# isi-vista/VistaOCR

Hardware: AMD Instinct MI355X
Metric: line-images/sec (train, batch 32, 30x600 grey) (higher is better)
Workload: dtype f32 (the LSTM's large GEMMs as bf16x6 products: fp32 operands split exactly into three bf16 planes, six bf16 MFMAs per fp32 product, fp32 accumulate; VOCR_LSTM_GEMM=f32 restores the f32-MFMA kernels); 1 GPU; configs[1]: 32 synthetic 1x30x600 grey lines per GPU, 20 labels/line, V=96, 3xBiLSTM-512, train() = H2D of the batch + fwd+CTC+bwd+allreduce+clamp+Adam, loss returned as a float; widths=600 .. 600 px, mean 600, conv_dtype=fp32, global_batch=32, parallelism=dp1, ranks_seen=1, backend=none, per_rank_rng=seed 1234 + 1000*rank after an identical init

## Files before the change

include/vocr.h:

```cpp
#ifndef VOCR_H
#define VOCR_H
#include <stddef.h>
#include <stdint.h>

#ifdef __cplusplus
extern "C" {
#endif

#define VOCR_OK          0
#define VOCR_EINVAL     -1
#define VOCR_ELAUNCH    -2
#define VOCR_ENODEVICE  -3
#define VOCR_ECOMM      -4


const char* vocr_last_error(void);
#define VOCR_ABI_VERSION 5
int  vocr_abi_version(void);
int  vocr_profile_range_push(const char* name);
int  vocr_profile_range_pop(void);
int  vocr_device_count(void);

int vocr_conv3x3_pack_weights(const float* w, float* wpack_fwd, float* wpack_dgrad, int cout, int cin, void* stream);
int vocr_conv3x3_fwd(const float* x, const float* wpack, const float* bias, float* y,
                     int n, int cin, int h, int w, int cout, void* stream);
size_t vocr_conv3x3_wgrad_workspace_bytes(int n, int cin, int h, int w, int cout);
int vocr_conv3x3_wgrad(const float* x, const float* dy, float* dw, void* workspace,
                       int n, int cin, int h, int w, int cout, void* stream);
int vocr_conv3x3_wino_supported(int cin, int cout);
size_t vocr_conv3x3_wino_pack_floats(int cout, int cin);
int vocr_conv3x3_wino_pack_weights(const float* w, float* wpack_fwd, float* wpack_dgrad, int cout, int cin, void* stream);
int vocr_conv3x3_wino_plan(int n, int cin, int h, int w, int cout);
int vocr_conv3x3_wino_fwd(const float* x, const float* wpack, const float* bias, float* y,
                          int n, int cin, int h, int w, int cout, void* stream);
size_t vocr_conv3x3_wgrad_wino_workspace_bytes(int n, int cin, int h, int w, int cout);
int vocr_conv3x3_wgrad_wino(const float* x, const float* dy, float* dw, void* workspace,
                            int n, int cin, int h, int w, int cout, void* stream);
int vocr_conv3x3_c1_fwd(const float* x, const float* w, const float* bias, float* y, int n, int h, int wd, int cout, int round_f16,
                        void* stream);
size_t vocr_conv3x3_c1_wgrad_workspace_bytes(int n, int h, int cout);
int vocr_conv3x3_c1_wgrad(const float* x, const float* dy, float* dw, float* dbias, void* workspace, int n, int h, int wd, int cout,
                          void* stream);
size_t vocr_conv3x3_f16_pack_bytes(int cout, int cin, int dgrad);
int vocr_conv3x3_f16_pack_weights(const float* w, void* wpack_fwd, void* wpack_dgrad, int cout, int cin, void* stream);
int vocr_conv3x3_f16_fwd(const float* x, const void* wpack, const float* bias, float* y,
                         int n, int cin, int h, int w, int cout, void* stream);
int vocr_conv3x3_wgrad_f16(const float* x, const float* dy, float* dw, void* workspace,
                           int n, int cin, int h, int w, int cout, void* stream);
int vocr_conv3x3_h16_supported(int cin, int cout);
int vocr_conv3x3_h16_plan(int n, int cin, int h, int w, int cout);
int vocr_conv3x3_h16_fwd(const void* x16, const void* wpack, const float* bias, float* y,
                         int n, int cin, int h, int w, int cout, void* stream);
int vocr_f16_padded_row(int w);
int vocr_f32_to_f16_layouts(const float* x, void* nhwc, void* nchwp, int n, int c, int h, int w, void* stream);
int vocr_conv3x3_wgrad_h16_supported(int cin, int cout);
size_t vocr_conv3x3_wgrad_h16_workspace_bytes(int n, int cin, int h, int w, int cout);
int vocr_conv3x3_wgrad_h16(const void* x16p, const void* dy16p, float* dw, void* workspace,
                           int n, int cin, int h, int w, int cout, void* stream);
size_t vocr_channel_sum_workspace_bytes(int n, int c, int hw);
int vocr_channel_sum(const float* x, float* out, int n, int c, int hw, void* workspace, void* stream);

size_t vocr_bn_workspace_bytes(int n, int c, int hw);
int vocr_bn_train_stats(const float* y, int n, int c, int hw, float eps, float momentum,
                        float* mean, float* invstd, float* running_mean, float* running_var,
                        int64_t* num_batches_tracked, float* xhat_sum, void* workspace, void* stream);
int vocr_bn_eval_stats(const float* running_mean, const float* running_var, int c, float eps,
                       float* mean, float* invstd, void* stream);
int vocr_bn_relu_apply(const float* y, const float* mean, const float* invstd, const float* gamma,
                       const float* beta, float* out, int n, int c, int hw, void* stream);
int vocr_bn_train_relu_apply(const float* y, const float* gamma, const float* beta, float* out, int n, int c, int hw, float eps,
                             float momentum, float* mean, float* invstd, float* running_mean, float* running_var,
                             int64_t* num_batches_tracked, float* xhat_sum, void* workspace, void* stream);
int vocr_bn_train_relu_fracpool2x2_fwd(const float* y, const float* gamma, const float* beta, const float* samples, float* out,
                                       int32_t* idx, int n, int c, int h, int w, int oh, int ow, float eps, float momentum,
                                       float* mean, float* invstd, float* running_mean, float* running_var,
                                       int64_t* num_batches_tracked, float* xhat_sum, void* workspace, void* stream);
int vocr_bn_relu_bwd(const float* da, const float* y, const float* mean, const float* invstd,
                     const float* gamma, const float* beta, const float* xhat_sum, float* dy, float* dgamma, float* dbeta,
                     float* dconv_bias, int n, int c, int hw, void* workspace, void* stream);

int vocr_fracpool2x2_fwd(const float* x, const float* samples, float* out, int32_t* idx,
                         int n, int c, int h, int w, int oh, int ow, void* stream);
int vocr_bn_relu_fracpool2x2_fwd(const float* y, const float* mean, const float* invstd, const float* gamma,
                                 const float* beta, const float* samples, float* out, int32_t* idx,
                                 int n, int c, int h, int w, int oh, int ow, void* stream);
int vocr_bn_relu_fracpool2x2_bwd_supported(int h, int w, int oh, int ow);
int vocr_bn_relu_fracpool2x2_bwd(const float* dout, const int32_t* idx, const float* samples, const float* y,
                                 const float* mean, const float* invstd, const float* gamma, const float* beta,
                                 const float* xhat_sum, float* dy, float* dgamma, float* dbeta, float* dconv_bias,
                                 int n, int c, int h, int w, int oh, int ow, void* workspace, void* stream);
int vocr_fracpool2x2_bwd(const float* dout, const int32_t* idx, float* dx,
                         int n, int c, int h, int w, int oh, int ow, void* stream);

int vocr_relu_maxpool2_fwd(const float* x, float* out, int32_t* idx, int n, int c, int h, int w, void* stream);
int vocr_relu_maxpool2_bwd(const float* dout, const float* out, const int32_t* idx, float* dx,
                           int n, int c, int h, int w, void* stream);

size_t vocr_gemm_workspace_bytes(int m, int n, int k, int has_bias_or_relu);
int vocr_gemm(int transa, int transb, int m, int n, int k,
              const float* a, int lda, const float* b, int ldb, float* c, int ldc,
              const float* bias, int relu, int accumulate, void* workspace, size_t workspace_bytes, void* stream);
#define VOCR_GEMM_PLAN_INTS 12
int vocr_gemm_plan(int transa, int transb, int m, int n, int k, int lda, int ldb, int ldc, int aligned, int has_bias_or_relu,
                   int accumulate, size_t workspace_bytes, int nprob, int nseg, int tiles_only, int* plan);
size_t vocr_gemm_pair_workspace_bytes(int m, int n, int k, int mode);
int vocr_gemm_pair(int mode, int transa, int transb, int m, int n, int k, const float* a0, const float* a1, int lda,
                   const float* b0, const float* b1, int ldb, float* c0, float* c1, int ldc, const float* bias0, const float* bias1,
                   int relu, void* workspace, size_t workspace_bytes, void* stream);
size_t vocr_colsum_workspace_bytes(int m, int n);
int vocr_colsum(const float* x, float* out, int m, int n, void* workspace, void* stream);
int vocr_relu_bwd(const float* dy, const float* out, float* dz, size_t count, void* stream);
int vocr_bchw_to_wbch(const float* x, float* out, int b, int c, int h, int w, void* stream);
int vocr_wbch_to_bchw(const float* x, float* out, int b, int c, int h, int w, void* stream);
int vocr_mul(const float* x, const float* mask, float* out, size_t count, void* stream);
int vocr_add(const float* x, const float* y, float* out, size_t count, void* stream);
int vocr_scale_dev(const float* x, const float* scalar, float* out, size_t count, void* stream);
int vocr_dropout_fwd(const float* x, float* out, float* mask, size_t count, float p, uint64_t seed, void* stream);
int vocr_dropout_mask(float* mask, size_t count, float p, uint64_t seed, void* stream);

size_t vocr_lstm_workspace_bytes(int t, int b, int h);
int vocr_lstm_fwd(const float* xproj, const float* whh_fwd, const float* whh_rev, const int32_t* lens, float* y,
                  float* gates, float* cell, void* workspace, int t, int b, int h, int32_t* health, void* stream);
int vocr_lstm_fwd_range(const float* xproj, const float* whh_fwd, const float* whh_rev, const int32_t* lens, float* y,
                        float* gates, float* cell, void* workspace, int t, int b, int h, int step_begin, int step_end,
                        int32_t* health, void* stream);
int vocr_lstm_bwd(const float* dy, const float* whht_fwd, const float* whht_rev, const int32_t* lens, const float* gates,
                  const float* cell, float* dgates, void* workspace, int t, int b, int h, int32_t* health, void* stream);
int vocr_lstm_bwd_bias(const float* dy, const float* whht_fwd, const float* whht_rev, const int32_t* lens, const float* gates,
                       const float* cell, float* dgates, float* dbias, void* workspace, int t, int b, int h, int32_t* health,
                       void* stream);
int vocr_lstm_bwd_parts_supported(int t, int b, int h);
int vocr_lstm_bwd_parts(const float* dy, const float* dy_mask, const float* whht_fwd, const float* whht_rev, const int32_t* lens,
                        const float* gates, const float* cell, float* dgates, void* workspace, int t, int b, int h,
                        int32_t* health, void* stream);
int vocr_lstm_bias_from_parts(float* dbias, const void* workspace, int t, int b, int h, void* stream);

size_t vocr_gemm_x6_planes_bytes(int rows, int k);
int vocr_gemm_x6_split(const float* x, const float* x2, int seg, int seg_axis, const float* mask, long ld, int rows, int k, int k_contiguous,
                       void* planes, void* stream);
size_t vocr_gemm_x6_workspace_bytes(int m, int n, int k);
#define VOCR_GEMM_X6_PLAN_INTS 9
int vocr_gemm_x6_plan(int m, int n, int k, int b_rows, int b_row0, int b_row0_2, int has_workspace, int* plan);
int vocr_gemm_x6(const void* a_planes, int a_rows, int a_k, int a_row0, int a_kk0, const void* b_planes, int b_rows, int b_k, int b_row0, int b_kk0,
                 int m, int n, int k, float* c0, float* c1, int csplit, int rsplit, int ldc, const float* bias0, const float* bias1, int relu,
                 void* workspace, void* stream);

int vocr_gemm_x6_two_views(const void* a_planes, int a_rows, int a_k, int a_row0, const void* b_planes, int b_rows, int b_k, int m, int n, int k,
                           int rsplit, int a_kk0, int b_row0, int b_kk0, int a_kk0_2, int b_row0_2, int b_kk0_2, float* c0, float* c1, int ldc,
                           void* workspace, void* stream);

size_t vocr_gemm_h3_planes_bytes(int rows, int k);
int vocr_gemm_h3_split(const float* x, const float* x2, int seg, int seg_axis, const float* mask, long ld, int rows, int k, int k_contiguous,
                       float bound, void* planes, void* stream);
int vocr_gemm_h3(const void* a_planes, int a_rows, int a_k, int a_row0, int a_kk0, const void* b_planes, int b_rows, int b_k, int b_row0, int b_kk0,
                 int m, int n, int k, float* c0, float* c1, int csplit, int rsplit, int ldc, const float* bias0, const float* bias1, int relu,
                 void* workspace, void* stream);
int vocr_gemm_h3_two_views(const void* a_planes, int a_rows, int a_k, int a_row0, const void* b_planes, int b_rows, int b_k, int m, int n, int k,
                           int rsplit, int a_kk0, int b_row0, int b_kk0, int a_kk0_2, int b_row0_2, int b_kk0_2, float* c0, float* c1, int ldc,
                           void* workspace, void* stream);

int vocr_lstm_packed_supported(int b, int h);
int vocr_seq_rowmap(const int32_t* lens, int t, int b, int rows, int32_t* to_packed, int32_t* to_dense, void* stream);
int vocr_gather_rows(const float* src, float* dst, const int32_t* map, long nrows, int n, const float* fill, void* stream);
size_t vocr_gather_rows_fill_grad_workspace_bytes(int n);
int vocr_gather_rows_fill_grad(const float* dout, const int32_t* map, long nrows, int n, float* dfill, void* workspace, void* stream);
int vocr_lstm_fwd_packed(const float* xproj, const float* whh_fwd, const float* whh_rev, const int32_t* lens, float* y,
                         float* gates, float* cell, void* workspace, int t, int b, int h, int rows, int32_t* health, void* stream);
int vocr_lstm_bwd_packed(const float* dy, const float* dy_mask, const float* whht_fwd, const float* whht_rev, const int32_t* lens,
                         const float* gates, const float* cell, float* dgates, float* dbias, void* workspace, int t, int b, int h,
                         int rows, int32_t* health, void* stream);

int vocr_lstm_follow_supported(int b, int h);
size_t vocr_lstm_xproj_pack_bytes(int h);
int vocr_lstm_xproj_pack(const float* w_ih_fwd, const float* w_ih_rev, float* wpack, int h, void* stream);
int vocr_lstm_fwd_lead(const float* xproj, const float* xproj2, const float* whh_fwd, const float* whh_rev, const int32_t* lens,
                       float* y, float* gates, float* cell, void* workspace, int t, int b, int h, int rows,
                       const float* next_wpack, const float* next_bias, const float* y_mask, float* next_planes,
                       int32_t* health, void* stream);

size_t vocr_ctc_workspace_bytes(int t, int b, int v, int max_label_len);
int vocr_ctc_loss_grad(const float* logits, const int32_t* labels, const int32_t* label_offsets,
                       const int32_t* label_lens, const int32_t* act_lens, float* nll, float* dlogits,
                       void* workspace, int t, int b, int v, int max_label_len, void* stream);

int vocr_argmax_rows(const float* x, int32_t* idx, float* maxv, int rows, int v, void* stream);
int vocr_greedy_collapse(const int32_t* idx, const float* maxv, const int32_t* lens, const int32_t* canon,
                         int32_t* out_labels, int32_t* out_counts, int t, int b, float thresh, void* stream);

size_t vocr_ctc_beam_workspace_bytes(int t, int b, int v, int beam, int nbest);
int vocr_ctc_beam_search(const float* logits, const int32_t* lens, int t, int b, int v, const int32_t* canon, int beam, int nbest,
                         const float* lm_logp, const int32_t* lm_next, const float* lm_eos, int lm_states, int lm_start,
                         float lm_weight, float insertion_bonus, float prune_logp, int32_t* out_labels, int32_t* out_lens,
                         float* out_scores, void* workspace, size_t workspace_bytes, void* stream);

size_t vocr_ctc_word_beam_workspace_bytes(int t, int b, int v, int beam, int nbest);
int vocr_ctc_word_beam_search(const float* logits, const int32_t* lens, int t, int b, int v, const int32_t* canon, int beam, int nbest,
                              const int32_t* cls_kind, const int32_t* cls_tok, const int32_t* trie_next, const int32_t* trie_tok,
                              const float* trie_la, int trie_nodes, const int32_t* lm_off, const int32_t* lm_succ_tok,
                              const float* lm_succ_logp, const int32_t* lm_succ_next, const float* lm_bow, const int32_t* lm_back,
                              int lm_states, int lm_succ, int lm_tokens, int lm_start, int tok_unk, int tok_eos, float lm_weight,
                              float word_bonus, float oov_penalty, int32_t* out_labels, int32_t* out_lens, float* out_scores,
                              void* workspace, size_t workspace_bytes, void* stream);

size_t vocr_ctc_align_workspace_bytes(int t, int b, int v, int n, int max_label_len);
int vocr_ctc_align(const float* logits, const int32_t* lens, int t, int b, int v, const int32_t* canon,
                   const int32_t* labels, const int32_t* label_lens, int n, int label_stride, int max_label_len,
                   float* out_scores, int32_t* out_spans, float* out_label_scores,
                   void* workspace, size_t workspace_bytes, void* stream);

size_t vocr_ctc_edit_workspace_bytes(int t, int b, int v, int n, int max_label_len);
int vocr_ctc_edit_scores(const float* logits, const int32_t* lens, int t, int b, int v, const int32_t* canon,
                         const int32_t* labels, const int32_t* label_lens, int n, int label_stride, int max_label_len,
                         float* out_ctc, float* out_sub, float* out_del, float* out_ins,
                         void* workspace, size_t workspace_bytes, void* stream);

size_t vocr_ctc_nbest_workspace_bytes(int t, int b, int v, int n, int max_label_len);
int vocr_ctc_nbest_grad(const float* logits, const int32_t* lens, int t, int b, int v, const int32_t* canon,
                        const int32_t* labels, const int32_t* label_lens, int n, int label_stride, int max_label_len,
                        const float* weights, float* out_ctc, float* dlogits,
                        void* workspace, size_t workspace_bytes, void* stream);

size_t vocr_ctc_keyword_workspace_bytes(int t, int b, int v, int nq, int max_query_len);
int vocr_ctc_keyword_scores(const float* logits, const int32_t* lens, int t, int b, int v, const int32_t* canon,
                            const int32_t* queries, const int32_t* query_lens, const int32_t* query_flags, int nq, int query_stride,
                            int max_query_len, float* out_log_count, float* out_best, int32_t* out_span,
                            void* workspace, size_t workspace_bytes, void* stream);

size_t vocr_ctc_grammar_workspace_bytes(int t, int b, int v, int g, int max_states, int max_arcs, int want_best);
int vocr_ctc_grammar_scores(const float* logits, const int32_t* lens, int t, int b, int v, const int32_t* canon,
// ... 47 lines not shown
```

vistaocr_amd/_lib.py:

```python
import ctypes
import os
from ctypes import c_char_p, c_float, c_int, c_size_t, c_uint32, c_uint64, c_void_p

_HERE = os.path.dirname(os.path.abspath(__file__))
LIB_PATH = os.path.join(_HERE, "csrc", "libvocr.so")

P, I, F, Z, U64, U32 = c_void_p, c_int, c_float, c_size_t, c_uint64, c_uint32

SIGNATURES = {
    "vocr_last_error": (c_char_p, []),
    "vocr_abi_version": (I, []),
    "vocr_device_count": (I, []),
    "vocr_profile_range_push": (I, [c_char_p]),
    "vocr_profile_range_pop": (I, []),
    "vocr_conv3x3_pack_weights": (I, [P, P, P, I, I, P]),
    "vocr_conv3x3_fwd": (I, [P, P, P, P, I, I, I, I, I, P]),
    "vocr_conv3x3_wgrad_workspace_bytes": (Z, [I, I, I, I, I]),
    "vocr_conv3x3_wgrad": (I, [P, P, P, P, I, I, I, I, I, P]),
    "vocr_conv3x3_wino_supported": (I, [I, I]),
    "vocr_conv3x3_wino_pack_floats": (Z, [I, I]),
    "vocr_conv3x3_wino_pack_weights": (I, [P, P, P, I, I, P]),
    "vocr_conv3x3_wino_fwd": (I, [P, P, P, P, I, I, I, I, I, P]),
    "vocr_conv3x3_wino_plan": (I, [I, I, I, I, I]),
    "vocr_conv3x3_wgrad_wino_workspace_bytes": (Z, [I, I, I, I, I]),
    "vocr_conv3x3_wgrad_wino": (I, [P, P, P, P, I, I, I, I, I, P]),
    "vocr_conv3x3_f16_pack_bytes": (Z, [I, I, I]),
    "vocr_conv3x3_f16_pack_weights": (I, [P, P, P, I, I, P]),
    "vocr_conv3x3_f16_fwd": (I, [P, P, P, P, I, I, I, I, I, P]),
    "vocr_conv3x3_wgrad_f16": (I, [P, P, P, P, I, I, I, I, I, P]),
    "vocr_conv3x3_c1_fwd": (I, [P, P, P, P, I, I, I, I, I, P]),
    "vocr_conv3x3_c1_wgrad_workspace_bytes": (Z, [I, I, I]),
    "vocr_conv3x3_c1_wgrad": (I, [P, P, P, P, P, I, I, I, I, P]),
    "vocr_conv3x3_h16_supported": (I, [I, I]),
    "vocr_conv3x3_h16_plan": (I, [I, I, I, I, I]),
    "vocr_conv3x3_h16_fwd": (I, [P, P, P, P, I, I, I, I, I, P]),
    "vocr_f16_padded_row": (I, [I]),
    "vocr_f32_to_f16_layouts": (I, [P, P, P, I, I, I, I, P]),
    "vocr_conv3x3_wgrad_h16_supported": (I, [I, I]),
    "vocr_conv3x3_wgrad_h16_workspace_bytes": (Z, [I, I, I, I, I]),
    "vocr_conv3x3_wgrad_h16": (I, [P, P, P, P, I, I, I, I, I, P]),
    "vocr_channel_sum_workspace_bytes": (Z, [I, I, I]),
    "vocr_channel_sum": (I, [P, P, I, I, I, P, P]),
    "vocr_bn_workspace_bytes": (Z, [I, I, I]),
    "vocr_bn_train_stats": (I, [P, I, I, I, F, F, P, P, P, P, P, P, P, P]),
    "vocr_bn_eval_stats": (I, [P, P, I, F, P, P, P]),
    "vocr_bn_relu_apply": (I, [P, P, P, P, P, P, I, I, I, P]),
    "vocr_bn_train_relu_apply": (I, [P, P, P, P, I, I, I, F, F, P, P, P, P, P, P, P, P]),
    "vocr_bn_train_relu_fracpool2x2_fwd": (I, [P, P, P, P, P, P, I, I, I, I, I, I, F, F, P, P, P, P, P, P, P, P]),
    "vocr_bn_relu_bwd": (I, [P, P, P, P, P, P, P, P, P, P, P, I, I, I, P, P]),
    "vocr_bn_relu_fracpool2x2_bwd_supported": (I, [I, I, I, I]),
    "vocr_bn_relu_fracpool2x2_bwd": (I, [P] * 13 + [I] * 6 + [P, P]),
    "vocr_fracpool2x2_fwd": (I, [P, P, P, P, I, I, I, I, I, I, P]),
    "vocr_bn_relu_fracpool2x2_fwd": (I, [P, P, P, P, P, P, P, P, I, I, I, I, I, I, P]),
    "vocr_fracpool2x2_bwd": (I, [P, P, P, I, I, I, I, I, I, P]),
    "vocr_relu_maxpool2_fwd": (I, [P, P, P, I, I, I, I, P]),
    "vocr_relu_maxpool2_bwd": (I, [P, P, P, P, I, I, I, I, P]),
    "vocr_gemm_workspace_bytes": (Z, [I, I, I, I]),
    "vocr_gemm": (I, [I, I, I, I, I, P, I, P, I, P, I, P, I, I, P, Z, P]),
    "vocr_gemm_plan": (I, [I, I, I, I, I, I, I, I, I, I, I, Z, I, I, I, P]),
    "vocr_gemm_pair_workspace_bytes": (Z, [I, I, I, I]),
    "vocr_gemm_pair": (I, [I, I, I, I, I, I, P, P, I, P, P, I, P, P, I, P, P, I, P, Z, P]),
    "vocr_gemm_x6_planes_bytes": (Z, [I, I]),
    "vocr_gemm_x6_split": (I, [P, P, I, I, P, ctypes.c_long, I, I, I, P, P]),
    "vocr_gemm_x6_workspace_bytes": (Z, [I, I, I]),
    "vocr_gemm_x6_plan": (I, [I, I, I, I, I, I, I, P]),
    "vocr_gemm_x6": (I, [P, I, I, I, I, P, I, I, I, I, I, I, I, P, P, I, I, I, P, P, I, P, P]),
    "vocr_gemm_x6_two_views": (I, [P, I, I, I, P, I, I, I, I, I, I, I, I, I, I, I, I, P, P, I, P, P]),
    "vocr_gemm_h3_two_views": (I, [P, I, I, I, P, I, I, I, I, I, I, I, I, I, I, I, I, P, P, I, P, P]),
    "vocr_gemm_h3_planes_bytes": (Z, [I, I]),
    "vocr_gemm_h3_split": (I, [P, P, I, I, P, ctypes.c_long, I, I, I, ctypes.c_float, P, P]),
    "vocr_gemm_h3": (I, [P, I, I, I, I, P, I, I, I, I, I, I, I, P, P, I, I, I, P, P, I, P, P]),
    "vocr_colsum_workspace_bytes": (Z, [I, I]),
    "vocr_colsum": (I, [P, P, I, I, P, P]),
    "vocr_relu_bwd": (I, [P, P, P, Z, P]),
    "vocr_bchw_to_wbch": (I, [P, P, I, I, I, I, P]),
    "vocr_wbch_to_bchw": (I, [P, P, I, I, I, I, P]),
    "vocr_mul": (I, [P, P, P, Z, P]),
    "vocr_add": (I, [P, P, P, Z, P]),
    "vocr_scale_dev": (I, [P, P, P, Z, P]),
    "vocr_dropout_fwd": (I, [P, P, P, Z, F, U64, P]),
    "vocr_dropout_mask": (I, [P, Z, F, U64, P]),
    "vocr_lstm_workspace_bytes": (Z, [I, I, I]),
    "vocr_lstm_fwd": (I, [P, P, P, P, P, P, P, P, I, I, I, P, P]),
    "vocr_lstm_fwd_range": (I, [P, P, P, P, P, P, P, P, I, I, I, I, I, P, P]),
    "vocr_lstm_bwd": (I, [P, P, P, P, P, P, P, P, I, I, I, P, P]),
    "vocr_lstm_bwd_bias": (I, [P, P, P, P, P, P, P, P, P, I, I, I, P, P]),
    "vocr_lstm_bwd_parts_supported": (I, [I, I, I]),
    "vocr_lstm_bwd_parts": (I, [P, P, P, P, P, P, P, P, P, I, I, I, P, P]),
    "vocr_lstm_bias_from_parts": (I, [P, P, I, I, I, P]),
    "vocr_lstm_packed_supported": (I, [I, I]),
    "vocr_seq_rowmap": (I, [P, I, I, I, P, P, P]),
    "vocr_gather_rows": (I, [P, P, P, ctypes.c_long, I, P, P]),
    "vocr_gather_rows_fill_grad_workspace_bytes": (Z, [I]),
    "vocr_gather_rows_fill_grad": (I, [P, P, ctypes.c_long, I, P, P, P]),
    "vocr_lstm_fwd_packed": (I, [P, P, P, P, P, P, P, P, I, I, I, I, P, P]),
    "vocr_lstm_follow_supported": (I, [I, I]),
    "vocr_lstm_xproj_pack_bytes": (Z, [I]),
    "vocr_lstm_xproj_pack": (I, [P, P, P, I, P]),
    "vocr_lstm_fwd_lead": (I, [P, P, P, P, P, P, P, P, P, I, I, I, I, P, P, P, P, P, P]),
    "vocr_lstm_bwd_packed": (I, [P, P, P, P, P, P, P, P, P, P, I, I, I, I, P, P]),
    "vocr_ctc_workspace_bytes": (Z, [I, I, I, I]),
    "vocr_ctc_loss_grad": (I, [P, P, P, P, P, P, P, P, I, I, I, I, P]),
    "vocr_argmax_rows": (I, [P, P, P, I, I, P]),
    "vocr_greedy_collapse": (I, [P, P, P, P, P, P, I, I, F, P]),
    "vocr_ctc_beam_workspace_bytes": (Z, [I, I, I, I, I]),
    "vocr_ctc_beam_search": (I, [P, P, I, I, I, P, I, I, P, P, P, I, I, F, F, F, P, P, P, P, Z, P]),
    "vocr_ctc_word_beam_workspace_bytes": (Z, [I, I, I, I, I]),
    "vocr_ctc_word_beam_search": (I, [P, P, I, I, I, P, I, I, P, P, P, P, P, I, P, P, P, P, P, P, I, I, I, I, I, I, F, F, F, P, P, P, P,
                                      Z, P]),
    "vocr_ctc_align_workspace_bytes": (Z, [I, I, I, I, I]),
    "vocr_ctc_align": (I, [P, P, I, I, I, P, P, P, I, I, I, P, P, P, P, Z, P]),
    "vocr_ctc_edit_workspace_bytes": (Z, [I, I, I, I, I]),
    "vocr_ctc_edit_scores": (I, [P, P, I, I, I, P, P, P, I, I, I, P, P, P, P, P, Z, P]),
    "vocr_ctc_nbest_workspace_bytes": (Z, [I, I, I, I, I]),
    "vocr_ctc_nbest_grad": (I, [P, P, I, I, I, P, P, P, I, I, I, P, P, P, P, Z, P]),
    "vocr_ctc_keyword_workspace_bytes": (Z, [I, I, I, I, I]),
    "vocr_ctc_keyword_scores": (I, [P, P, I, I, I, P, P, P, P, I, I, I, P, P, P, P, Z, P]),
    "vocr_ctc_grammar_workspace_bytes": (Z, [I, I, I, I, I, I, I]),
    "vocr_ctc_grammar_scores": (I, [P, P, I, I, I, P, P, P, I, P, P, P, P, I, I, P, P, P, P, I, P, Z, P]),
    "vocr_ctc_grammar_grad_workspace_bytes": (Z, [I, I, I, I, I, I, I]),
    "vocr_ctc_grammar_grad": (I, [P, P, I, I, I, P, P, P, I, P, P, P, P, I, I, P, P, P, P, P, Z, P]),
    "vocr_edit_stats_workspace_bytes": (Z, [I, I, I, I, I, I, I]),
    "vocr_edit_stats": (I, [P, P, I, I, I, P, P, I, I, I, P, I, P, P, I, I, P, P, P, I, P, Z, P]),
    "vocr_augment_workspace_bytes": (Z, [I, I, I, I]),
    "vocr_augment_lines": (I, [P, P, I, I, I, I, P, P, I, I, I, P, P, Z, P]),
    "vocr_ctc_entropy_workspace_bytes": (Z, [I, I, I, I, I]),
    "vocr_ctc_entropy": (I, [P, P, I, I, I, P, P, P, I, I, P, P, P, P, P, Z, P]),
    "vocr_clamp_adam": (I, [P, P, P, P, Z, F, F, F, F, F, F, F, I, P, P]),
    "vocr_clamp": (I, [P, Z, F, P, P]),
    "vocr_comm_unique_id": (I, [P]),
    "vocr_comm_create": (I, [ctypes.POINTER(P), P, I, I, I]),
    "vocr_allreduce_sum_f32": (I, [P, P, Z, P]),
    "vocr_comm_destroy": (I, [P]),
}

ABI_VERSION = 5

_lib = None


def load():
    global _lib
    if _lib is not None:
        return _lib
    if not os.path.exists(LIB_PATH):
        raise RuntimeError("libvocr.so not found at %s — run `python -m vistaocr_amd.build` (needs hipcc). "
                           "vistaocr_amd has no CPU fallback." % LIB_PATH)
    lib = ctypes.CDLL(LIB_PATH)
    lib.vocr_abi_version.restype = ctypes.c_int
    got = lib.vocr_abi_version()
    if got != ABI_VERSION:
        raise RuntimeError("libvocr.so at %s answers ABI version %d, this package was written for %d (include/vocr.h: VOCR_ABI_VERSION) "
                           "— a stale binary; rebuild with `python -m vistaocr_amd.build --force`" % (LIB_PATH, got, ABI_VERSION))
    for name, (res, args) in SIGNATURES.items():
        fn = getattr(lib, name)
        fn.restype = res
        fn.argtypes = args
    _lib = lib
    return lib


def check(rc, what):
    if rc != 0:
        msg = load().vocr_last_error()
        raise RuntimeError("%s failed (%d): %s" % (what, rc, msg.decode() if msg else "?"))


_TIMED = None
_FILTER = {}


def enable_timing(names, keep=False):
    global _TIMED, _FILTER
    old = _TIMED if keep and _TIMED is not None else {}
    if not names:
        _TIMED = {k: v for k, v in old.items()} if (keep and old) else None
        _FILTER = {k: (lambda a: False) for k in (_TIMED or {})}
        return
    _FILTER = dict(names) if isinstance(names, dict) else {n: None for n in names}
    _TIMED = {n: old.get(n, []) for n in _FILTER}


def timing_records():
    return _TIMED or {}


def call(name, *args):
    if _TIMED is not None and name in _TIMED and (_FILTER.get(name) is None or _FILTER[name](args)):
        import torch
        e0 = torch.cuda.Event(enable_timing=True)
        e1 = torch.cuda.Event(enable_timing=True)
        e0.record()
        rc = getattr(load(), name)(*args)
        e1.record()
        _TIMED[name].append((args, e0, e1))
    else:
        rc = getattr(load(), name)(*args)
    if rc != 0:
        check(rc, name)


# ... 17 lines not shown
```

vistaocr_amd/csrc/bn_pool.hip:

```cpp
#include "vocr_common.h"

namespace {

constexpr int BN_CHUNK_ELEMS = 16384;

__host__ __device__ inline int bn_nchunk(long per_channel) {
    long n = (per_channel + BN_CHUNK_ELEMS - 1) / BN_CHUNK_ELEMS;
    return (int)(n < 1 ? 1 : (n > 512 ? 512 : n));
}

__device__ __forceinline__ long chan_addr(long e, int c, int C, long HW) {
    const long n = e / HW, r = e - n * HW;
    return (n * C + c) * HW + r;
}

struct ChanWalk {
    long n;
    long r;
    __device__ __forceinline__ ChanWalk(long e, long HW) : n(e / HW), r(e - (e / HW) * HW) {}
    __device__ __forceinline__ long addr(int c, int C, long HW) const { return (n * C + c) * HW + r; }
    __device__ __forceinline__ void advance(long step, long HW) {
        r += step;
        while (r >= HW) { r -= HW; ++n; }
    }
};

__device__ __forceinline__ void block_reduce2(double& a, double& b, double* red) {
    a = wave_sum_d(a);
    b = wave_sum_d(b);
    const int wave = threadIdx.x >> 6;
    if ((threadIdx.x & 63) == 0) { red[wave * 2] = a; red[wave * 2 + 1] = b; }
    __syncthreads();
    a = (red[0] + red[2]) + (red[4] + red[6]);
    b = (red[1] + red[3]) + (red[5] + red[7]);
}

template <int V> struct VecT { typedef float type __attribute__((ext_vector_type(V))); };
template <> struct VecT<1> { typedef float type; };
template <int V> __device__ __forceinline__ float vget(const typename VecT<V>::type& v, int i) { return v[i]; }
template <> __device__ __forceinline__ float vget<1>(const float& v, int) { return v; }
template <int V> __device__ __forceinline__ void vset(typename VecT<V>::type& v, int i, float x) { v[i] = x; }
template <> __device__ __forceinline__ void vset<1>(float& v, int, float x) { v = x; }

template <int V>
__global__ __launch_bounds__(256) void bn_stats_partial_kernel(const float* __restrict__ y, double* __restrict__ part,
                                                               int N, int C, long HW, int nchunk, long per) {
    typedef typename VecT<V>::type vec;
    __shared__ double red[8];
    const int c = blockIdx.x, j = blockIdx.y;
    const long total = (long)N * HW;
    const long beg = j * per, end = min(total, beg + per);
    double s = 0.0, q = 0.0;
    ChanWalk wk(beg + (long)threadIdx.x * V, HW);
    for (long e = beg + (long)threadIdx.x * V; e < end; e += 256 * V, wk.advance(256 * V, HW)) {
        const vec v = *(const vec*)(y + wk.addr(c, C, HW));
#pragma unroll
        for (int i = 0; i < V; ++i) {
            const double x = (double)vget<V>(v, i);
            s += x;
            q += x * x;
        }
    }
    block_reduce2(s, q, red);
    if (threadIdx.x == 0) {
        part[((long)c * nchunk + j) * 2] = s;
        part[((long)c * nchunk + j) * 2 + 1] = q;
    }
}

__global__ void bn_stats_final_kernel(const double* __restrict__ part, int C, int nchunk, long count, float eps,
                                      float momentum, float* __restrict__ mean, float* __restrict__ invstd,
                                      float* __restrict__ rmean, float* __restrict__ rvar, long long* __restrict__ nbt,
                                      float* __restrict__ xhat_sum) {
    const int c = blockIdx.x * blockDim.x + threadIdx.x;
    if (c == 0 && nbt) *nbt += 1;
    if (c >= C) return;
    double s = 0.0, q = 0.0;
    for (int j = 0; j < nchunk; ++j) {
        s += part[((long)c * nchunk + j) * 2];
        q += part[((long)c * nchunk + j) * 2 + 1];
    }
    const double m = s / (double)count;
    double var = q / (double)count - m * m;
    if (var < 0.0) var = 0.0;
    mean[c] = (float)m;
    invstd[c] = (float)(1.0 / sqrt(var + (double)eps));
    if (xhat_sum) xhat_sum[c] = (float)((s - (double)count * (double)mean[c]) * (double)invstd[c]);
    if (rmean) rmean[c] = (1.f - momentum) * rmean[c] + momentum * (float)m;
    if (rvar) {
        const double unbiased = count > 1 ? var * (double)count / (double)(count - 1) : var;
        rvar[c] = (1.f - momentum) * rvar[c] + momentum * (float)unbiased;
    }
}

__global__ void bn_eval_stats_kernel(const float* __restrict__ rmean, const float* __restrict__ rvar, int C, float eps,
                                     float* __restrict__ mean, float* __restrict__ invstd) {
    const int c = blockIdx.x * blockDim.x + threadIdx.x;
    if (c >= C) return;
    mean[c] = rmean[c];
    invstd[c] = 1.0f / sqrtf(rvar[c] + eps);
}

constexpr int BN_MAX_CHUNKS = 512;
__device__ __forceinline__ void combine_partials(const double* __restrict__ part, int c, int nchunk, double* stage ,
                                                 double& s, double& q) {
    for (int j = threadIdx.x; j < nchunk; j += blockDim.x) {
        stage[2 * j] = part[((long)c * nchunk + j) * 2];
        stage[2 * j + 1] = part[((long)c * nchunk + j) * 2 + 1];
    }
    __syncthreads();
    if (threadIdx.x == 0) {
        double a = 0.0, b = 0.0;
        for (int j = 0; j < nchunk; ++j) {
            a += stage[2 * j];
            b += stage[2 * j + 1];
        }
        stage[2 * BN_MAX_CHUNKS] = a;
        stage[2 * BN_MAX_CHUNKS + 1] = b;
    }
    __syncthreads();
    s = stage[2 * BN_MAX_CHUNKS];
    q = stage[2 * BN_MAX_CHUNKS + 1];
}

__device__ __forceinline__ void bn_train_stats_of(double s, double q, long count, float eps, float momentum, int c, bool writer,
                                                  float* __restrict__ mean, float* __restrict__ invstd, float* __restrict__ rmean,
                                                  float* __restrict__ rvar, long long* __restrict__ nbt, float* __restrict__ xhat_sum,
                                                  float& mu, float& is) {
    const double m = s / (double)count;
    double var = q / (double)count - m * m;
    if (var < 0.0) var = 0.0;
    mu = (float)m;
    is = (float)(1.0 / sqrt(var + (double)eps));
    if (writer && threadIdx.x == 0) {
        if (c == 0 && nbt) *nbt += 1;
        mean[c] = mu;
        invstd[c] = is;
        if (xhat_sum) xhat_sum[c] = (float)((s - (double)count * (double)mu) * (double)is);
        if (rmean) rmean[c] = (1.f - momentum) * rmean[c] + momentum * (float)m;
        if (rvar) {
            const double unbiased = count > 1 ? var * (double)count / (double)(count - 1) : var;
            rvar[c] = (1.f - momentum) * rvar[c] + momentum * (float)unbiased;
        }
    }
}

struct BnFusedStats {
    const double* part;
    int nchunk;
    long count;
    float eps, momentum;
    float *mean, *invstd, *rmean, *rvar, *xhat_sum;
    long long* nbt;
};

template <int V>
__global__ __launch_bounds__(256) void bn_relu_apply_kernel(const float* __restrict__ y, const float* __restrict__ mean,
                                                            const float* __restrict__ invstd,
                                                            const float* __restrict__ gamma,
                                                            const float* __restrict__ beta, float* __restrict__ out,
                                                            int C, long HW, BnFusedStats fs) {
    typedef typename VecT<V>::type vec;
    __shared__ double stage[2 * BN_MAX_CHUNKS + 2];
    const long plane = blockIdx.y;
    const int c = (int)(plane % C);
    float mu, is;
    if (fs.part) {
        double s_, q_;
        combine_partials(fs.part, c, fs.nchunk, stage, s_, q_);
        bn_train_stats_of(s_, q_, fs.count, fs.eps, fs.momentum, c, blockIdx.x == 0 && plane < C, fs.mean, fs.invstd, fs.rmean, fs.rvar, fs.nbt,
                          fs.xhat_sum, mu, is);
    } else {
        mu = mean[c];
        is = invstd[c];
    }
    const float g = gamma[c], b = beta[c];
    const vec* yp = (const vec*)(y + plane * HW);
    vec* op = (vec*)(out + plane * HW);
    const long nv = HW / V;
    for (long i = (long)blockIdx.x * 256 + threadIdx.x; i < nv; i += (long)gridDim.x * 256) {
        const vec in = yp[i];
        vec o;
#pragma unroll
        for (int k = 0; k < V; ++k) {
            const float v = (vget<V>(in, k) - mu) * is * g + b;
            vset<V>(o, k, v > 0.f ? v : 0.f);
        }
        op[i] = o;
    }
}

template <int V>
__global__ __launch_bounds__(256) void bn_bwd_partial_kernel(const float* __restrict__ da, const float* __restrict__ y,
                                                             const float* __restrict__ mean,
                                                             const float* __restrict__ invstd,
                                                             const float* __restrict__ gamma,
                                                             const float* __restrict__ beta, double* __restrict__ part,
                                                             int N, int C, long HW, int nchunk, long per) {
    typedef typename VecT<V>::type vec;
    __shared__ double red[8];
    const int c = blockIdx.x, j = blockIdx.y;
    const float mu = mean[c], is = invstd[c], g = gamma[c], b = beta[c];
    const long total = (long)N * HW;
    const long beg = j * per, end = min(total, beg + per);
    double s1 = 0.0, s2 = 0.0;
    __builtin_amdgcn_s_setprio(3);
    constexpr int U = 4;
    ChanWalk wk(beg + (long)threadIdx.x * V, HW);
    for (long e = beg + (long)threadIdx.x * V; e < end; e += (long)U * 256 * V) {
        vec yv[U], dv[U];
        bool ok[U];
        const long a0 = wk.addr(c, C, HW);
#pragma unroll
        for (int u = 0; u < U; ++u) {
            ok[u] = e + (long)u * 256 * V < end;
            const long a = ok[u] ? wk.addr(c, C, HW) : a0;
            yv[u] = *(const vec*)(y + a);
            dv[u] = *(const vec*)(da + a);
            wk.advance(256 * V, HW);
        }
#pragma unroll
        for (int u = 0; u < U; ++u) {
            float p1 = 0.f, p2 = 0.f;
#pragma unroll
            for (int k = 0; k < V; ++k) {
                const float xh = (vget<V>(yv[u], k) - mu) * is;
                const float o = xh * g + b;
                const float dz = o > 0.f ? vget<V>(dv[u], k) : 0.f;
                p1 += dz;
                p2 += dz * xh;
            }
            if (ok[u]) {
                s1 += (double)p1;
                s2 += (double)p2;
            }
        }
    }
    block_reduce2(s1, s2, red);
    if (threadIdx.x == 0) {
        part[((long)c * nchunk + j) * 2] = s1;
        part[((long)c * nchunk + j) * 2 + 1] = s2;
    }
}

__global__ __launch_bounds__(256) void bn_pool_bwd_partial_kernel(const float* __restrict__ dout, const int32_t* __restrict__ idx,
                                                                  const float* __restrict__ y, const float* __restrict__ mean,
                                                                  const float* __restrict__ invstd, const float* __restrict__ gamma,
                                                                  const float* __restrict__ beta, double* __restrict__ part, int N,
                                                                  int C, long HW, long OP, int nchunk, long per) {
    __shared__ double red[8];
    const int c = blockIdx.x, j = blockIdx.y;
    const float mu = mean[c], is = invstd[c], g = gamma[c], b = beta[c];
    const long total = (long)N * OP;
    const long beg = j * per, end = min(total, beg + per);
    double s1 = 0.0, s2 = 0.0;
    long wn[4], wr[4];
#pragma unroll
    for (int u = 0; u < 4; ++u) {
        const long e0 = beg + threadIdx.x + 256 * u;
        wn[u] = e0 / OP;
        wr[u] = e0 - wn[u] * OP;
    }
    for (long e = beg + threadIdx.x; e < end; e += 1024) {
        float d[4], yv[4];
        int ix[4];
        bool ok[4];
        long pl[4];
#pragma unroll
        for (int u = 0; u < 4; ++u) {
            ok[u] = e + 256 * u < end;
            pl[u] = (ok[u] ? wn[u] : 0) * C + c;
            const long r = ok[u] ? wr[u] : 0;
            d[u] = dout[pl[u] * OP + r];
            ix[u] = idx[pl[u] * OP + r];
        }
// ... 222 lines not shown
    }
}

__global__ __launch_bounds__(256) void bn_pool_bwd_apply_kernel(const float* __restrict__ dout, const int32_t* __restrict__ idx,
                                                                const float* __restrict__ samples, const float* __restrict__ y,
                                                                const float* __restrict__ mean, const float* __restrict__ invstd,
                                                                const float* __restrict__ gamma, const float* __restrict__ beta,
                                                                float* __restrict__ dgamma, float* __restrict__ dbeta,
                                                                float* __restrict__ dy, int C, int H, int W, int OH, int OW,
                                                                float alpha_h, float alpha_w, float inv_count, const double* __restrict__ part,
                                                                int nchunk, double inv_count_d, const float* __restrict__ xhat_sum,
                                                                float* __restrict__ dconv_bias) {
    __shared__ double stage[2 * BN_MAX_CHUNKS + 2];
    extern __shared__ int inv[];
    int* wa = inv;
    int* wb = inv + W + 4;
    int* ha = inv + 2 * W + 8;
    int* hb = inv + 2 * W + 8 + H;
    const long plane = blockIdx.x;
    const int c = (int)(plane % C);
    const int tid = threadIdx.x;
    const float uw = samples[plane * 2], uh = samples[plane * 2 + 1];
    for (int i = tid; i < 2 * W + 8 + 2 * H; i += 256) inv[i] = -1;
    __syncthreads();
    for (int o = tid; o < OW - 1; o += 256) {
        const int st = frac_start(o, uw, alpha_w, W, OW);
        wa[st] = o;
        wb[st + 1] = o;
    }
    for (int o = tid; o < OH - 1; o += 256) {
        const int st = frac_start(o, uh, alpha_h, H, OH);
        ha[st] = o;
        hb[st + 1] = o;
    }
    __syncthreads();
    const float mu = mean[c], is = invstd[c], g = gamma[c], b = beta[c];
    double s1, s2;
    combine_partials(part, c, nchunk, stage, s1, s2);
    const float dbeta_c = (float)s1, dgamma_c = (float)s2;
    if (plane < C && tid == 0) {
        dbeta[c] = dbeta_c;
        dgamma[c] = dgamma_c;
        if (dconv_bias) dconv_bias[c] = xhat_sum ? (float)(-(double)g * (double)is * (s2 * inv_count_d) * (double)xhat_sum[c]) : 0.f;
    }
    const float k1 = dbeta_c * inv_count, k2 = dgamma_c * inv_count, gs = g * is;
    const float* dp = dout + plane * (long)OH * OW;
    const int32_t* ip = idx + plane * (long)OH * OW;
    const f32x4* yp = (const f32x4*)(y + plane * (long)H * W);
    f32x4* op = (f32x4*)(dy + plane * (long)H * W);
    const int GW = W >> 2, G = H * GW;
    for (int gi = tid; gi < G; gi += 256) {
        const int h = gi / GW, w0 = (gi - h * GW) << 2;
        const f32x4 yv = yp[gi];
        const int orow[2] = {ha[h], hb[h]};
        const int ocol[5] = {wb[w0], wa[w0], wa[w0 + 1], wa[w0 + 2], wa[w0 + 3]};
        float da[4] = {0.f, 0.f, 0.f, 0.f};
        const int p0 = h * W + w0;
#pragma unroll
        for (int r = 0; r < 2; ++r) {
            if (!__any(orow[r] >= 0)) continue;
            int wi[5];
            float wd[5];
#pragma unroll
            for (int k = 0; k < 5; ++k) {
                const int o = max(orow[r], 0) * OW + max(ocol[k], 0);
                wi[k] = ip[o];
                wd[k] = dp[o];
            }
#pragma unroll
            for (int k = 0; k < 5; ++k) {
                const bool ok = orow[r] >= 0 && ocol[k] >= 0;
                const int j = wi[k] - p0;
#pragma unroll
                for (int q = 0; q < 4; ++q) da[q] += (ok && j == q) ? wd[k] : 0.f;
            }
        }
        if (h >= H - 2 || w0 + 3 >= W - 2) {
            const int lr = h >= H - 2 ? OH - 1 : -1, lc = w0 + 3 >= W - 2 ? OW - 1 : -1;
#pragma unroll
            for (int r = 0; r < 3; ++r) {
                const int orr = r < 2 ? orow[r] : lr;
#pragma unroll
                for (int k = 0; k < 6; ++k) {
                    const int occ = k < 5 ? ocol[k] : lc;
                    if ((r < 2 && k < 5) || orr < 0 || occ < 0) continue;
                    const int o = orr * OW + occ;
                    const int j = ip[o] - p0;
                    if (j >= 0 && j < 4) da[j] += dp[o];
                }
            }
        }
        f32x4 ov;
#pragma unroll
        for (int q = 0; q < 4; ++q) {
            const float xh = (yv[q] - mu) * is;
            const float act = xh * g + b;
            const float dz = act > 0.f ? da[q] : 0.f;
            ov[q] = gs * (dz - k1 - xh * k2);
        }
        op[gi] = ov;
    }
}

__global__ __launch_bounds__(256) void relu_maxpool2_fwd_kernel(const float* __restrict__ x, float* __restrict__ out,
                                                                int32_t* __restrict__ idx, int H, int W, int OH, int OW) {
    const long plane = blockIdx.y;
    const float* xp = x + plane * (long)H * W;
    const int total = OH * OW;
    for (int o = blockIdx.x * 256 + threadIdx.x; o < total; o += gridDim.x * 256) {
        const int oh = o / OW, ow = o % OW;
        int best = (2 * oh) * W + 2 * ow;
        float mv = -INFINITY;
#pragma unroll
        for (int dh = 0; dh < 2; ++dh)
#pragma unroll
            for (int dw = 0; dw < 2; ++dw) {
                const int p = (2 * oh + dh) * W + 2 * ow + dw;
                const float v = fmaxf(xp[p], 0.f);
                if (v > mv) { mv = v; best = p; }
            }
        out[plane * total + o] = mv;
        idx[plane * total + o] = best;
    }
}

__global__ __launch_bounds__(256) void relu_maxpool2_bwd_kernel(const float* __restrict__ dout, const float* __restrict__ out,
                                                                const int32_t* __restrict__ idx, float* __restrict__ dx,
                                                                long in_plane, int out_plane) {
    const long plane = blockIdx.y;
    for (int o = blockIdx.x * 256 + threadIdx.x; o < out_plane; o += gridDim.x * 256) {
        const long oi = plane * out_plane + o;
        dx[plane * in_plane + idx[oi]] = out[oi] > 0.f ? dout[oi] : 0.f;
    }
}

}

static inline int vec_width(int hw, const void* a, const void* b) {
    const uintptr_t m = (uintptr_t)a | (uintptr_t)b;
    if (hw % 4 == 0 && (m & 15) == 0) return 4;
    if (hw % 2 == 0 && (m & 7) == 0) return 2;
    return 1;
}
static inline long chunk_len(long per_channel, int nchunk) {
    const long per = (per_channel + nchunk - 1) / nchunk;
    return (per + 3) / 4 * 4;
}

extern "C" size_t vocr_bn_workspace_bytes(int n, int c, int hw) {
    if (n <= 0 || c <= 0 || hw <= 0) return 0;
    return (size_t)c * bn_nchunk((long)n * hw) * 2 * sizeof(double);
}

extern "C" int vocr_bn_train_stats(const float* y, int n, int c, int hw, float eps, float momentum, float* mean,
                                   float* invstd, float* running_mean, float* running_var, int64_t* num_batches_tracked,
                                   float* xhat_sum, void* workspace, void* stream) {
    VOCR_CHECK_ARG(y && mean && invstd && workspace && n > 0 && c > 0 && hw > 0, "vocr_bn_train_stats: bad argument");
    hipStream_t s = (hipStream_t)stream;
    const int nchunk = bn_nchunk((long)n * hw);
    const int V = vec_width(hw, y, y);
    const long per = chunk_len((long)n * hw, nchunk);
    if (V == 4) bn_stats_partial_kernel<4><<<dim3(c, nchunk), 256, 0, s>>>(y, (double*)workspace, n, c, hw, nchunk, per);
    else if (V == 2) bn_stats_partial_kernel<2><<<dim3(c, nchunk), 256, 0, s>>>(y, (double*)workspace, n, c, hw, nchunk, per);
    else bn_stats_partial_kernel<1><<<dim3(c, nchunk), 256, 0, s>>>(y, (double*)workspace, n, c, hw, nchunk, per);
    VOCR_CHECK_LAUNCH("vocr_bn_train_stats(partial)");
    bn_stats_final_kernel<<<vocr_cdiv(c, 64), 64, 0, s>>>((const double*)workspace, c, nchunk, (long)n * hw, eps, momentum,
                                                          mean, invstd, running_mean, running_var, (long long*)num_batches_tracked, xhat_sum);
    VOCR_CHECK_LAUNCH("vocr_bn_train_stats(final)");
    return VOCR_OK;
}

extern "C" int vocr_bn_eval_stats(const float* running_mean, const float* running_var, int c, float eps, float* mean,
                                  float* invstd, void* stream) {
    VOCR_CHECK_ARG(running_mean && running_var && mean && invstd && c > 0, "vocr_bn_eval_stats: bad argument");
    bn_eval_stats_kernel<<<vocr_cdiv(c, 64), 64, 0, (hipStream_t)stream>>>(running_mean, running_var, c, eps, mean, invstd);
    VOCR_CHECK_LAUNCH("vocr_bn_eval_stats");
    return VOCR_OK;
}

static inline dim3 plane_grid(long planes, long per_plane) {
    long gx = (per_plane + 1023) / 1024;
    if (gx < 1) gx = 1;
    if (gx > 64) gx = 64;
    return dim3((unsigned)gx, (unsigned)planes);
}

extern "C" int vocr_bn_relu_apply(const float* y, const float* mean, const float* invstd, const float* gamma,
                                  const float* beta, float* out, int n, int c, int hw, void* stream) {
    VOCR_CHECK_ARG(y && mean && invstd && gamma && beta && out && n > 0 && c > 0 && hw > 0, "vocr_bn_relu_apply: bad argument");
    VOCR_CHECK_ARG((long)n * c <= 65535, "vocr_bn_relu_apply: n*c > 65535 planes");
    const int V = vec_width(hw, y, out);
    const dim3 grid = plane_grid((long)n * c, hw / V);
    const BnFusedStats none = {nullptr, 0, 0, 0.f, 0.f, nullptr, nullptr, nullptr, nullptr, nullptr, nullptr};
    if (V == 4) bn_relu_apply_kernel<4><<<grid, 256, 0, (hipStream_t)stream>>>(y, mean, invstd, gamma, beta, out, c, hw, none);
    else if (V == 2) bn_relu_apply_kernel<2><<<grid, 256, 0, (hipStream_t)stream>>>(y, mean, invstd, gamma, beta, out, c, hw, none);
    else bn_relu_apply_kernel<1><<<grid, 256, 0, (hipStream_t)stream>>>(y, mean, invstd, gamma, beta, out, c, hw, none);
    VOCR_CHECK_LAUNCH("vocr_bn_relu_apply");
    return VOCR_OK;
}

namespace {
int bn_launch_partial(const float* y, int n, int c, int hw, void* workspace, hipStream_t s, int* nchunk_out) {
    const int nchunk = bn_nchunk((long)n * hw);
    const int V = vec_width(hw, y, y);
    const long per = chunk_len((long)n * hw, nchunk);
    if (V == 4) bn_stats_partial_kernel<4><<<dim3(c, nchunk), 256, 0, s>>>(y, (double*)workspace, n, c, hw, nchunk, per);
    else if (V == 2) bn_stats_partial_kernel<2><<<dim3(c, nchunk), 256, 0, s>>>(y, (double*)workspace, n, c, hw, nchunk, per);
    else bn_stats_partial_kernel<1><<<dim3(c, nchunk), 256, 0, s>>>(y, (double*)workspace, n, c, hw, nchunk, per);
    *nchunk_out = nchunk;
    return VOCR_OK;
}
}

extern "C" int vocr_bn_train_relu_apply(const float* y, const float* gamma, const float* beta, float* out, int n, int c, int hw, float eps,
                                        float momentum, float* mean, float* invstd, float* running_mean, float* running_var,
                                        int64_t* num_batches_tracked, float* xhat_sum, void* workspace, void* stream) {
    VOCR_CHECK_ARG(y && gamma && beta && out && mean && invstd && workspace && n > 0 && c > 0 && hw > 0, "vocr_bn_train_relu_apply: bad argument");
    VOCR_CHECK_ARG((long)n * c <= 65535, "vocr_bn_train_relu_apply: n*c > 65535 planes");
    hipStream_t s = (hipStream_t)stream;
    int nchunk = 0;
    bn_launch_partial(y, n, c, hw, workspace, s, &nchunk);
    VOCR_CHECK_LAUNCH("vocr_bn_train_relu_apply(partial)");
    const BnFusedStats fs = {(const double*)workspace, nchunk, (long)n * hw, eps, momentum, mean, invstd, running_mean, running_var, xhat_sum,
                             (long long*)num_batches_tracked};
    const int V = vec_width(hw, y, out);
    const dim3 grid = plane_grid((long)n * c, hw / V);
    if (V == 4) bn_relu_apply_kernel<4><<<grid, 256, 0, s>>>(y, mean, invstd, gamma, beta, out, c, hw, fs);
    else if (V == 2) bn_relu_apply_kernel<2><<<grid, 256, 0, s>>>(y, mean, invstd, gamma, beta, out, c, hw, fs);
    else bn_relu_apply_kernel<1><<<grid, 256, 0, s>>>(y, mean, invstd, gamma, beta, out, c, hw, fs);
    VOCR_CHECK_LAUNCH("vocr_bn_train_relu_apply(apply)");
    return VOCR_OK;
}

extern "C" int vocr_bn_relu_bwd(const float* da, const float* y, const float* mean, const float* invstd,
                                const float* gamma, const float* beta, const float* xhat_sum, float* dy, float* dgamma, float* dbeta,
                                float* dconv_bias, int n, int c, int hw, void* workspace, void* stream) {
    VOCR_CHECK_ARG(da && y && mean && invstd && gamma && beta && dy && dgamma && dbeta && workspace, "vocr_bn_relu_bwd: null pointer");
    VOCR_CHECK_ARG(n > 0 && c > 0 && hw > 0 && (long)n * c <= 65535, "vocr_bn_relu_bwd: bad shape");
    hipStream_t s = (hipStream_t)stream;
    const int nchunk = bn_nchunk((long)n * hw);
    const int V = (vec_width(hw, da, y) < vec_width(hw, dy, dy)) ? vec_width(hw, da, y) : vec_width(hw, dy, dy);
    const long per = chunk_len((long)n * hw, nchunk);
    if (V == 4) bn_bwd_partial_kernel<4><<<dim3(c, nchunk), 256, 0, s>>>(da, y, mean, invstd, gamma, beta, (double*)workspace, n, c, hw, nchunk, per);
    else if (V == 2) bn_bwd_partial_kernel<2><<<dim3(c, nchunk), 256, 0, s>>>(da, y, mean, invstd, gamma, beta, (double*)workspace, n, c, hw, nchunk, per);
    else bn_bwd_partial_kernel<1><<<dim3(c, nchunk), 256, 0, s>>>(da, y, mean, invstd, gamma, beta, (double*)workspace, n, c, hw, nchunk, per);
    VOCR_CHECK_LAUNCH("vocr_bn_relu_bwd(partial)");
    const dim3 grid = plane_grid((long)n * c, hw / V);
    const float inv_count = 1.0f / (float)((long)n * hw);
    const double inv_count_d = 1.0 / (double)((long)n * hw);
    const double* part = (const double*)workspace;
    if (V == 4) bn_bwd_apply_kernel<4><<<grid, 256, 0, s>>>(da, y, mean, invstd, gamma, beta, dgamma, dbeta, dy, c, hw, inv_count, part, nchunk, inv_count_d, xhat_sum, dconv_bias);
    else if (V == 2) bn_bwd_apply_kernel<2><<<grid, 256, 0, s>>>(da, y, mean, invstd, gamma, beta, dgamma, dbeta, dy, c, hw, inv_count, part, nchunk, inv_count_d, xhat_sum, dconv_bias);
    else bn_bwd_apply_kernel<1><<<grid, 256, 0, s>>>(da, y, mean, invstd, gamma, beta, dgamma, dbeta, dy, c, hw, inv_count, part, nchunk, inv_count_d, xhat_sum, dconv_bias);
    VOCR_CHECK_LAUNCH("vocr_bn_relu_bwd(apply)");
    return VOCR_OK;
}

extern "C" int vocr_bn_relu_fracpool2x2_bwd_supported(int h, int w, int oh, int ow) {
    if (h < 2 || w < 2 || oh < 2 || ow < 2 || oh > h - 1 || ow > w - 1) return 0;
    return ((float)(h - 2) / (float)(oh - 1) >= 1.01f && (float)(w - 2) / (float)(ow - 1) >= 1.01f && w % 4 == 0 &&
            (2 * w + 8 + 2 * h) * 4 <= 64 * 1024) ? 1 : 0;
}

extern "C" int vocr_bn_relu_fracpool2x2_bwd(const float* dout, const int32_t* idx, const float* samples, const float* y,
                                            const float* mean, const float* invstd, const float* gamma, const float* beta,
                                            const float* xhat_sum, float* dy, float* dgamma, float* dbeta, float* dconv_bias, int n,
                                            int c, int h, int w, int oh, int ow, void* workspace, void* stream) {
    VOCR_CHECK_ARG(dout && idx && samples && y && mean && invstd && gamma && beta && dy && dgamma && dbeta && workspace,
                   "vocr_bn_relu_fracpool2x2_bwd: null pointer");
    VOCR_CHECK_ARG(n > 0 && c > 0 && (long)n * c <= 65535 && vocr_bn_relu_fracpool2x2_bwd_supported(h, w, oh, ow),
                   "vocr_bn_relu_fracpool2x2_bwd: unsupported shape h=%d w=%d oh=%d ow=%d", h, w, oh, ow);
    hipStream_t s = (hipStream_t)stream;
    const long op = (long)oh * ow, hw = (long)h * w;
    const int nchunk = bn_nchunk((long)n * hw);
    const long per = ((long)n * op + nchunk - 1) / nchunk;
    bn_pool_bwd_partial_kernel<<<dim3(c, nchunk), 256, 0, s>>>(dout, idx, y, mean, invstd, gamma, beta, (double*)workspace, n, c, hw, op,
                                                              nchunk, per);
    VOCR_CHECK_LAUNCH("vocr_bn_relu_fracpool2x2_bwd(partial)");
    const float alpha_h = (float)(h - 2) / (float)(oh - 1), alpha_w = (float)(w - 2) / (float)(ow - 1);
    bn_pool_bwd_apply_kernel<<<(unsigned)(n * c), 256, (size_t)(2 * w + 8 + 2 * h) * sizeof(int), s>>>(
        dout, idx, samples, y, mean, invstd, gamma, beta, dgamma, dbeta, dy, c, h, w, oh, ow, alpha_h, alpha_w,
        1.0f / (float)((long)n * hw), (const double*)workspace, nchunk, 1.0 / (double)((long)n * hw), xhat_sum, dconv_bias);
    VOCR_CHECK_LAUNCH("vocr_bn_relu_fracpool2x2_bwd(apply)");
    return VOCR_OK;
}

extern "C" int vocr_fracpool2x2_fwd(const float* x, const float* samples, float* out, int32_t* idx, int n, int c, int h,
                                    int w, int oh, int ow, void* stream) {
    VOCR_CHECK_ARG(x && samples && out && idx, "vocr_fracpool2x2_fwd: null pointer");
    VOCR_CHECK_ARG(n > 0 && c > 0 && h >= 2 && w >= 2 && oh >= 1 && ow >= 1 && oh <= h - 1 && ow <= w - 1 && (long)n * c <= 65535,
                   "vocr_fracpool2x2_fwd: bad shape h=%d w=%d oh=%d ow=%d", h, w, oh, ow);
    const float alpha_h = oh > 1 ? (float)(h - 2) / (float)(oh - 1) : 0.f;
    const float alpha_w = ow > 1 ? (float)(w - 2) / (float)(ow - 1) : 0.f;
    fracpool_fwd_kernel<<<plane_grid((long)n * c, (long)oh * ow), 256, 0, (hipStream_t)stream>>>(x, samples, out, idx, h, w, oh,
                                                                                             ow, alpha_h, alpha_w);
    VOCR_CHECK_LAUNCH("vocr_fracpool2x2_fwd");
    return VOCR_OK;
}

extern "C" int vocr_bn_relu_fracpool2x2_fwd(const float* y, const float* mean, const float* invstd, const float* gamma,
                                            const float* beta, const float* samples, float* out, int32_t* idx, int n, int c,
                                            int h, int w, int oh, int ow, void* stream) {
    VOCR_CHECK_ARG(y && mean && invstd && gamma && beta && samples && out && idx, "vocr_bn_relu_fracpool2x2_fwd: null pointer");
    VOCR_CHECK_ARG(n > 0 && c > 0 && h >= 2 && w >= 2 && oh >= 1 && ow >= 1 && oh <= h - 1 && ow <= w - 1 && (long)n * c <= 65535,
                   "vocr_bn_relu_fracpool2x2_fwd: bad shape h=%d w=%d oh=%d ow=%d", h, w, oh, ow);
    const float alpha_h = oh > 1 ? (float)(h - 2) / (float)(oh - 1) : 0.f;
    const float alpha_w = ow > 1 ? (float)(w - 2) / (float)(ow - 1) : 0.f;
    const BnFusedStats none = {nullptr, 0, 0, 0.f, 0.f, nullptr, nullptr, nullptr, nullptr, nullptr, nullptr};
    bn_relu_fracpool_fwd_kernel<<<plane_grid((long)n * c, (long)oh * ow), 256, 0, (hipStream_t)stream>>>(
        y, mean, invstd, gamma, beta, samples, out, idx, c, h, w, oh, ow, alpha_h, alpha_w, none);
    VOCR_CHECK_LAUNCH("vocr_bn_relu_fracpool2x2_fwd");
    return VOCR_OK;
}

extern "C" int vocr_bn_train_relu_fracpool2x2_fwd(const float* y, const float* gamma, const float* beta, const float* samples, float* out,
                                                  int32_t* idx, int n, int c, int h, int w, int oh, int ow, float eps, float momentum,
                                                  float* mean, float* invstd, float* running_mean, float* running_var,
                                                  int64_t* num_batches_tracked, float* xhat_sum, void* workspace, void* stream) {
    VOCR_CHECK_ARG(y && gamma && beta && samples && out && idx && mean && invstd && workspace, "vocr_bn_train_relu_fracpool2x2_fwd: null pointer");
    VOCR_CHECK_ARG(n > 0 && c > 0 && h >= 2 && w >= 2 && oh >= 1 && ow >= 1 && oh <= h - 1 && ow <= w - 1 && (long)n * c <= 65535,
                   "vocr_bn_train_relu_fracpool2x2_fwd: bad shape h=%d w=%d oh=%d ow=%d", h, w, oh, ow);
    hipStream_t s = (hipStream_t)stream;
    int nchunk = 0;
    bn_launch_partial(y, n, c, h * w, workspace, s, &nchunk);
    VOCR_CHECK_LAUNCH("vocr_bn_train_relu_fracpool2x2_fwd(partial)");
    const BnFusedStats fs = {(const double*)workspace, nchunk, (long)n * h * w, eps, momentum, mean, invstd, running_mean, running_var, xhat_sum,
                             (long long*)num_batches_tracked};
    const float alpha_h = oh > 1 ? (float)(h - 2) / (float)(oh - 1) : 0.f;
    const float alpha_w = ow > 1 ? (float)(w - 2) / (float)(ow - 1) : 0.f;
    bn_relu_fracpool_fwd_kernel<<<plane_grid((long)n * c, (long)oh * ow), 256, 0, s>>>(y, mean, invstd, gamma, beta, samples, out, idx, c, h, w, oh, ow,
                                                                                       alpha_h, alpha_w, fs);
    VOCR_CHECK_LAUNCH("vocr_bn_train_relu_fracpool2x2_fwd(apply)");
    return VOCR_OK;
}

extern "C" int vocr_fracpool2x2_bwd(const float* dout, const int32_t* idx, float* dx, int n, int c, int h, int w, int oh,
                                    int ow, void* stream) {
    VOCR_CHECK_ARG(dout && idx && dx && n > 0 && c > 0 && (long)n * c <= 65535, "vocr_fracpool2x2_bwd: bad argument");
    hipStream_t s = (hipStream_t)stream;
    const long in_plane = (long)h * w;
    static const int use_lds = VOCR_EXPERIMENT_INT("VOCR_POOL_LDS", 1);
    if (use_lds && in_plane <= 8192) {
        pool_bwd_lds_kernel<8192><<<(unsigned)(n * c), 512, 0, s>>>(dout, idx, dx, (int)in_plane, oh * ow);
    } else if (use_lds && in_plane <= 18432) {
        pool_bwd_lds_kernel<18432><<<(unsigned)(n * c), 512, 0, s>>>(dout, idx, dx, (int)in_plane, oh * ow);
    } else if (use_lds && in_plane <= 36864) {
        pool_bwd_lds_kernel<36864><<<(unsigned)(n * c), 512, 0, s>>>(dout, idx, dx, (int)in_plane, oh * ow);
    } else {
        if (hipMemsetAsync(dx, 0, (size_t)n * c * in_plane * sizeof(float), s) != hipSuccess) {
            vocr_set_error("vocr_fracpool2x2_bwd: memset failed");
            return VOCR_ELAUNCH;
        }
        pool_bwd_scatter_kernel<<<plane_grid((long)n * c, (long)oh * ow), 256, 0, s>>>(dout, idx, dx, in_plane, oh * ow);
    }
    VOCR_CHECK_LAUNCH("vocr_fracpool2x2_bwd");
    return VOCR_OK;
}

extern "C" int vocr_relu_maxpool2_fwd(const float* x, float* out, int32_t* idx, int n, int c, int h, int w, void* stream) {
    VOCR_CHECK_ARG(x && out && idx && n > 0 && c > 0 && h >= 2 && w >= 2 && (long)n * c <= 65535, "vocr_relu_maxpool2_fwd: bad argument");
    const int oh = h / 2, ow = w / 2;
    relu_maxpool2_fwd_kernel<<<plane_grid((long)n * c, (long)oh * ow), 256, 0, (hipStream_t)stream>>>(x, out, idx, h, w, oh, ow);
    VOCR_CHECK_LAUNCH("vocr_relu_maxpool2_fwd");
    return VOCR_OK;
}

extern "C" int vocr_relu_maxpool2_bwd(const float* dout, const float* out, const int32_t* idx, float* dx, int n, int c,
                                      int h, int w, void* stream) {
    VOCR_CHECK_ARG(dout && out && idx && dx && n > 0 && c > 0 && (long)n * c <= 65535, "vocr_relu_maxpool2_bwd: bad argument");
    const int oh = h / 2, ow = w / 2;
    relu_maxpool2_bwd_kernel<<<plane_grid((long)n * c, (long)oh * ow), 256, 0, (hipStream_t)stream>>>(dout, out, idx, dx,
                                                                                                  (long)h * w, oh * ow);
    VOCR_CHECK_LAUNCH("vocr_relu_maxpool2_bwd");
    return VOCR_OK;
}
```

vistaocr_amd/csrc/conv_tail.h:

```cpp
#pragma once
#include "vocr_common.h"

namespace {

struct SegInfo { long base; int n; int h; int w0; int valid; int rows; int pw; int ow; };

template <int TAIL_WAVES>
__device__ __forceinline__ void conv3x3_tail_piece_px(float* __restrict__ red_, int pn, int ph, int pwc, bool pix_ok, bool live, int co_base,
                                                      const float* __restrict__ in, const float* __restrict__ wpack, const float* __restrict__ bias,
                                                      float* __restrict__ out, const float* __restrict__ zero_page, int Cin, int H, int W, int Cout) {
    float (*red)[16][64] = (float (*)[16][64])red_;
    const int tid = threadIdx.x, lane = tid & 63;
    const int wave = __builtin_amdgcn_readfirstlane(tid >> 6);
    const int li = lane & 31, lk = lane >> 5;
    (void)li;
    if (!live || co_base >= Cout) return;
    const long HW = (long)H * W;
    int toff[9];
    float tm[9];
#pragma unroll
    for (int t = 0; t < 9; ++t) {
        const int hh = ph + t / 3 - 1, ww = pwc + t % 3 - 1;
        tm[t] = (pix_ok && hh >= 0 && hh < H && ww >= 0 && ww < W) ? 1.f : 0.f;
        toff[t] = min(max(hh, 0), H - 1) * W + min(max(ww, 0), W - 1);
    }
    const float* xin = in + (long)pn * Cin * HW;
    const int co = co_base + (lane & 31);
    const bool co_ok = co < Cout;
    const int nsteps = (Cin + 2 * TAIL_WAVES - 1) / (2 * TAIL_WAVES);
    constexpr int DEPTH = 3;
    float a[DEPTH][9], b[DEPTH][9];
    auto loads = [&](int s, float (&av)[9], float (&bv)[9]) {
        const int ci = 2 * (TAIL_WAVES * s + wave) + lk;
        const bool ok = ci < Cin && s < nsteps;
        const float* wrow = (ok && co_ok) ? wpack + (long)ci * 9 * Cout + co : zero_page;
        const long wstride = (ok && co_ok) ? Cout : 0;
        const float* xc = xin + (long)min(ci, Cin - 1) * HW;
        const float cm = ok ? 1.f : 0.f;
#pragma unroll
        for (int t = 0; t < 9; ++t) {
            av[t] = wrow[t * wstride];
            bv[t] = xc[toff[t]] * (tm[t] * cm);
        }
    };
    f32x16 acc;
#pragma unroll
    for (int r = 0; r < 16; ++r) acc[r] = 0.f;
#pragma unroll
    for (int d = 0; d < DEPTH; ++d) loads(d, a[d], b[d]);
    for (int s0 = 0; s0 < nsteps; s0 += DEPTH) {
#pragma unroll
        for (int d = 0; d < DEPTH; ++d) {
            if (s0 + d < nsteps) {
#pragma unroll
                for (int t = 0; t < 9; ++t) acc = __builtin_amdgcn_mfma_f32_32x32x2f32(a[d][t], b[d][t], acc, 0, 0, 0);
                loads(s0 + d + DEPTH, a[d], b[d]);
            }
        }
    }
#pragma unroll
    for (int r = 0; r < 16; ++r) red[wave][r][lane] = acc[r];
    __syncthreads();
#pragma unroll
    for (int q = 0; q < 16 / TAIL_WAVES; ++q) {
        const int r = (16 / TAIL_WAVES) * wave + q;
        float sum = 0.f;
#pragma unroll
        for (int w8 = 0; w8 < TAIL_WAVES; ++w8) sum += red[w8][r][lane];
        const int oc = co_base + (r & 3) + 8 * (r >> 2) + 4 * lk;
        if (pix_ok && oc < Cout)
            out[(long)pn * Cout * HW + (long)oc * HW + (long)ph * W + pwc] = sum + (bias ? bias[oc] : 0.f);
    }
}

template <int TAIL_WAVES>
__device__ __forceinline__ void conv3x3_tail_piece_at(float* __restrict__ red_, const SegInfo& sg, int co_base, const float* __restrict__ in,
                                                      const float* __restrict__ wpack, const float* __restrict__ bias, float* __restrict__ out,
                                                      const float* __restrict__ zero_page, int Cin, int H, int W, int Cout) {
    const int li = threadIdx.x & 31;
    const int rr = li / sg.pw, cc = li - rr * sg.pw;
    conv3x3_tail_piece_px<TAIL_WAVES>(red_, sg.n, sg.h + rr, sg.w0 + cc, rr < sg.rows && cc < sg.ow, sg.valid != 0, co_base, in, wpack, bias, out,
                                      zero_page, Cin, H, W, Cout);
}

}
```

vistaocr_amd/csrc/conv_wino.hip:

```cpp
#include "vocr_common.h"
#include "conv_tail.h"

namespace {

constexpr int TS = 32;
constexpr int CI_H = 4;
constexpr int WR = CI_H * 12;
constexpr int PRW = 68;
constexpr int POFF = 34;
constexpr int PSEG = CI_H * 3 * PRW;

__device__ __attribute__((aligned(16))) float g_wino_zero_page[64];

__device__ __forceinline__ int xcd_slice_order(int b, int nwg) {
    const int x = b & 7, q = nwg >> 3, r = nwg & 7;
    return (x < r ? x * (q + 1) : r * (q + 1) + (x - r) * q) + (b >> 3);
}

__global__ void wino_pack_kernel(const float* __restrict__ w, float* __restrict__ pf, float* __restrict__ pd, int cout, int cin, int x4) {
    const int i = blockIdx.x * blockDim.x + threadIdx.x;
    const int total = cout * cin * 3;
    if (i >= total) return;
    const int kh = i % 3, ci = (i / 3) % cin, co = i / (3 * cin);
    const float* g = w + ((long)(co * cin + ci) * 3 + kh) * 3;
// ... 323 lines not shown
    auto store_patch = [&](int buf) __attribute__((always_inline)) {
#pragma unroll
        for (int j = 0; j < ROWS_W; ++j) P[buf * PBUF + j * PRW + m_lds] = rp[j];
        P[h_lane ? buf * PBUF + h_lds : DUMMY + lane] = rp[ROWS_W];
    };
    constexpr int IPR = CO_T / 64;
    unsigned w_vo[DPW];
#pragma unroll
    for (int d = 0; d < DPW; ++d) {
        const int q = wave + 4 * d, row = q / IPR, co = co0 + (q % IPR) * 64 + lane;
        w_vo[d] = co < Cout ? (unsigned)(row * Cout + co) * 16u : FAR;
    }
    auto dma_weights = [&](int ci0, int buf) __attribute__((always_inline)) {
#pragma unroll
        for (int d = 0; d < DPW; ++d)
            __builtin_amdgcn_raw_ptr_buffer_load_lds(w_rs, (__attribute__((address_space(3))) void*)(Wt + buf * WBUF + (wave + 4 * d) * 256), 16, w_vo[d],
                                                     ci0 * 3 * Cout * 16, 0, 0);
    };
    auto kloop = [&](int buf) __attribute__((always_inline)) {
        const float* wa = Wt + buf * WBUF + ((lk * 2 * 3) * CO_T + wco + li) * 4;
        const float* pb = P + buf * PBUF + wsg * PSEG + li + lk * 2 * 3 * PRW;
        f32x4 a[TM];
        f32x2 ev, ov;
        auto reads = [&](int s, f32x4 (&aa)[TM], f32x2& E, f32x2& O) __attribute__((always_inline)) {
            const int cp = s / 3, kh = s % 3;
            const float* pr = pb + (cp * 3 + kh) * PRW;
            E = f32x2{pr[0], pr[1]};
            O = f32x2{pr[POFF], pr[POFF + 1]};
#pragma unroll
            for (int i = 0; i < TM; ++i) aa[i] = *(const f32x4*)(wa + ((cp * 3 + kh) * CO_T + 32 * i) * 4);
        };
        reads(0, a, ev, ov);
#pragma unroll
        for (int s = 0; s < 6; ++s) {
            f32x4 an[TM];
            f32x2 ne = ev, no = ov;
#pragma unroll
            for (int i = 0; i < TM; ++i) an[i] = a[i];
            if (s + 1 < 6) reads(s + 1, an, ne, no);
            f32x2 v12;
            asm("v_pk_add_f32 %0, %1, %2 op_sel:[0,1] op_sel_hi:[0,1] neg_hi:[1,0]\n\ts_nop 1" : "=v"(v12) : "v"(ov), "v"(ev));
            const float vv[4] = {ev[0] - ev[1], v12[0], v12[1], ov[0] - ov[1]};
            __builtin_amdgcn_sched_barrier(0);
#pragma unroll
            for (int x = 0; x < 4; ++x)
#pragma unroll
                for (int i = 0; i < TM; ++i) acc[i][x] = __builtin_amdgcn_mfma_f32_32x32x2f32(a[i][x], vv[x], acc[i][x], 0, 0, 0);
#pragma unroll
            for (int i = 0; i < TM; ++i) a[i] = an[i];
            ev = ne; ov = no;
        }
    };

    const int nh = ((Cin + 2 * CI_H - 1) / (2 * CI_H)) * 2;
    dma_weights(0, 0);
    load_patch(0);
    store_patch(0);
    for (int h = 0; h < nh; h += 2) {
        __syncthreads();
        dma_weights((h + 1) * CI_H, 1);
        load_patch((h + 1) * CI_H);
        kloop(0);
        store_patch(1);
        __syncthreads();
        dma_weights((h + 2) * CI_H, 0);
        load_patch((h + 2) * CI_H);
        kloop(1);
        store_patch(0);
    }

    const WSlot os = wslot((seg0 + wsg) * TS + li, geo);
    const int px = 2 * os.k;
    if (!os.valid || os.k >= geo.T || px >= W) return;
    const bool two = px + 1 < W;
    float* obase = out + (long)os.n * Cout * HW + (long)os.h * W + px;
#pragma unroll
    for (int i = 0; i < TM; ++i)
#pragma unroll
        for (int r = 0; r < 16; ++r) {
            const int co = co0 + wco + i * 32 + (r & 3) + 8 * (r >> 2) + 4 * lk;
            if (co < Cout) {
                const float b = bias ? bias[co] : 0.f;
                const float m0 = acc[i][0][r], m1 = acc[i][1][r], m2 = acc[i][2][r], m3 = acc[i][3][r];
                float* o = obase + (long)co * HW;
                o[0] = ((m0 + m1) + m2) + b;
                if (two) o[1] = ((m1 - m2) - m3) + b;
            }
        }
}


__global__ __launch_bounds__(256, 2) void conv3x3_wino2_kernel_128(const float* __restrict__ in, const float* __restrict__ wpack, const float* __restrict__ bias,
                                                                   float* __restrict__ out, const float* __restrict__ zero_page, int N, int Cin, int H, int W, int Cout,
                                                                   WGeom geo, int co_tiles, const float* __restrict__ wdirect, int n_tail, int first_tail_tile) {
    conv3x3_wino2_body<128>(in, wpack, bias, out, zero_page, N, Cin, H, W, Cout, geo, co_tiles, wdirect, n_tail, first_tail_tile);
}
__global__ __launch_bounds__(256, 2) void conv3x3_wino2_kernel_64(const float* __restrict__ in, const float* __restrict__ wpack, const float* __restrict__ bias,
                                                                  float* __restrict__ out, const float* __restrict__ zero_page, int N, int Cin, int H, int W, int Cout,
                                                                  WGeom geo, int co_tiles, const float* __restrict__ wdirect, int n_tail, int first_tail_tile) {
    conv3x3_wino2_body<64>(in, wpack, bias, out, zero_page, N, Cin, H, W, Cout, geo, co_tiles, wdirect, n_tail, first_tail_tile);
}

#ifndef W43_CUT
#define W43_CUT 0
#endif
#ifndef W43_PACKED
#define W43_PACKED 1
#endif
constexpr int Q4_TS = 32;
constexpr int Q4_PRW = 132;
__global__ void wino4_pack_kernel(const float* __restrict__ w, float* __restrict__ pf, float* __restrict__ pd, int cout, int cin) {
    const int i = blockIdx.x * blockDim.x + threadIdx.x;
    const int total = cout * cin * 3;
    if (i >= total) return;
    const int kh = i % 3, ci = (i / 3) % cin, co = i / (3 * cin);
    const float* g = w + ((long)(co * cin + ci) * 3 + kh) * 3;
    auto put = [](float* p4, float* p2, float g0, float g1, float g2) {
        p4[0] = 0.25f * g0;
        p4[1] = -((g0 + g2) + g1) * (1.f / 6.f);
        p4[2] = -((g0 + g2) - g1) * (1.f / 6.f);
        p4[3] = (g0 * (1.f / 24.f) + g2 * (1.f / 6.f)) + g1 * (1.f / 12.f);
        p2[0] = (g0 * (1.f / 24.f) + g2 * (1.f / 6.f)) - g1 * (1.f / 12.f);
        p2[1] = g2;
    };
    if (pf) {
        float* p4 = pf + ((long)(ci * 3 + kh) * cout + co) * 4;
        float* p2 = pf + (long)cin * 3 * cout * 4 + ((long)(ci * 3 + kh) * cout + co) * 2;
        put(p4, p2, g[0], g[1], g[2]);
    }
    if (pd) {
        float* p4 = pd + ((long)(co * 3 + (2 - kh)) * cin + ci) * 4;
        float* p2 = pd + (long)cout * 3 * cin * 4 + ((long)(co * 3 + (2 - kh)) * cin + ci) * 2;
        put(p4, p2, g[2], g[1], g[0]);
    }
}

__device__ __forceinline__ void w43_input_xform(f32x2 e01, f32x2 e23, f32x2 e45, f32x2 ka, f32x2 kb, f32x2 kc, f32x2& v12, f32x2& v34,
                                                f32x2& v05) {
    f32x2 p2;
    asm("v_pk_fma_f32 %2, %4, %9, %6 op_sel:[0,0,0] op_sel_hi:[1,0,1]\n\t"
        "v_pk_fma_f32 %1, %5, %7, %6 op_sel:[0,0,0] op_sel_hi:[0,1,0]\n\t"
        "v_pk_fma_f32 %3, %4, %7, %5 op_sel:[1,0,1] op_sel_hi:[1,1,1]\n\t"
        "v_pk_fma_f32 %2, %5, %9, %2 op_sel:[0,1,0] op_sel_hi:[1,1,1]\n\t"
        "v_pk_add_f32 %0, %1, %3 op_sel:[0,0] op_sel_hi:[0,0] neg_hi:[0,1]\n\t"
        "v_pk_fma_f32 %1, %3, %8, %1 op_sel:[1,0,1] op_sel_hi:[1,1,1]\n\t"
        "s_nop 1"
        : "=&v"(v12), "=&v"(v34), "=&v"(v05), "=&v"(p2)
        : "v"(e01), "v"(e23), "v"(e45), "v"(ka), "v"(kb), "v"(kc));
}

template <int CO_T, int NW, int CS>
__device__ __forceinline__ void conv3x3_wino4_body(const float* __restrict__ in, const float* __restrict__ wpack, const float* __restrict__ bias,
                                                   float* __restrict__ out, const float* __restrict__ zero_page, int N, int Cin, int H, int W, int Cout,
                                                   WGeom geo, int co_tiles, const float* __restrict__ wdirect, int n_tail, int first_tail_tile) {
    constexpr int TM = 2, TN = 1;
    constexpr int WAVES_CO = CO_T / 64;
    constexpr int NSEG = NW / WAVES_CO;
    constexpr int RS = 3 * CS;
    constexpr int KS = RS / 2;
    constexpr int PSEG = RS * Q4_PRW;
    constexpr int ROWS_W = NSEG * RS / NW;
    constexpr int W4 = RS * CO_T * 4, W2 = RS * CO_T * 2;
    constexpr int WBUF = W4 + W2;
    constexpr int PBUF = NSEG * PSEG;
    constexpr int NDMA = WBUF / 256;
    constexpr int DPW = (NDMA + NW - 1) / NW;
    __shared__ __attribute__((aligned(16))) float lds[2 * WBUF + 2 * PBUF + 256 + 64];
    float* const Wt = lds;
    float* const P = lds + 2 * WBUF;
    constexpr int DMA_DUMMY = 2 * WBUF + 2 * PBUF, ST_DUMMY = DMA_DUMMY + 256;

    if ((int)blockIdx.x < n_tail) {
        constexpr int COSUB = CO_T / 32, PPW = COSUB * 4 * NSEG;
        const int piece = blockIdx.x, vt = first_tail_tile + piece / PPW, sub = piece % PPW;
        const int pb = sub / COSUB, q0 = ((vt / co_tiles) * NSEG + pb / 4) * Q4_TS + (pb & 3) * 8;
        const int pli = threadIdx.x & 31;
        const WSlot ps = wslot(q0 + (pli >> 2), geo);
        const int pcol = 4 * ps.k + (pli & 3);
        conv3x3_tail_piece_px<NW>(lds, ps.n, ps.h, pcol, ps.valid && ps.k < geo.T && pcol < W, q0 < geo.nslot,
                                 (vt % co_tiles) * CO_T + (sub % COSUB) * 32, in, wdirect, bias, out, zero_page, Cin, H, W, Cout);
        return;
    }
    const int tid = threadIdx.x, lane = tid & 63;
    const int wave = __builtin_amdgcn_readfirstlane(tid >> 6);
    const int li = lane & 31, lk = lane >> 5;
    const int v = xcd_slice_order(blockIdx.x - n_tail, gridDim.x - n_tail);
    const int co0 = (v % co_tiles) * CO_T;
    const int wco = (wave / NSEG) * 64, wsg = wave % NSEG;
    const int sega = (v / co_tiles) * NSEG;
    const int seg0 = sega + wsg;
    const int iHW = H * W;

    f32x16 acc[TM][TN][6];
#pragma unroll
    for (int i = 0; i < TM; ++i)
#pragma unroll
        for (int n = 0; n < TN; ++n)
#pragma unroll
            for (int x = 0; x < 6; ++x)
#pragma unroll
                for (int r = 0; r < 16; ++r) acc[i][n][x][r] = 0.f;

    constexpr unsigned FAR = 0x80000000u;
    const __amdgpu_buffer_rsrc_t in_rs = __builtin_amdgcn_make_buffer_rsrc((void*)in, 0, (int)((long)N * Cin * iHW * 4), 0x00020000);
    const __amdgpu_buffer_rsrc_t null_rs = __builtin_amdgcn_make_buffer_rsrc((void*)in, 0, 0, 0x00020000);
    const __amdgpu_buffer_rsrc_t w_rs = __builtin_amdgcn_make_buffer_rsrc((void*)wpack, 0, Cin * 18 * Cout * 4, 0x00020000);
    const int st_seg = (wave * ROWS_W) / RS, c_first = (wave * ROWS_W) % RS;
    unsigned m_vo[2][3];
#pragma unroll
    for (int hlf = 0; hlf < 2; ++hlf) {
        const int r = lane + 64 * hlf;
        const WSlot ms = wslot((sega + st_seg) * Q4_TS + (r >> 2), geo);
        const int col = 4 * ms.k - 1 + (r & 3);
        const bool ok = ms.valid && col >= 0 && col < W;
#pragma unroll
        for (int kh = 0; kh < 3; ++kh) {
            const int hh = ms.h + kh - 1;
            m_vo[hlf][kh] = (ok && hh >= 0 && hh < H) ? (unsigned)(ms.n * Cin * iHW + hh * W + col) * 4u : FAR;
        }
    }
    const int hj = min(lane >> 1, ROWS_W - 1), h_c = (c_first + hj) / 3, h_kh = (c_first + hj) % 3;
    const bool h_lane = lane < 2 * ROWS_W;
    unsigned h_vo;
    {
        const WSlot hs = wslot((sega + st_seg) * Q4_TS + 32, geo);
        const int col = 4 * hs.k - 1 + (lane & 1), hh = hs.h + h_kh - 1;
        h_vo = (hs.valid && h_lane && col >= 0 && col < W && hh >= 0 && hh < H) ? (unsigned)(hs.n * Cin * iHW + h_c * iHW + hh * W + col) * 4u : FAR;
    }
    const int p_rows = wave * ROWS_W * Q4_PRW;
    float rh;
    auto load_patch = [&](int ci0, int buf) __attribute__((always_inline)) {
        float* pp = P + buf * PBUF + p_rows;
#pragma unroll
        for (int j = 0; j < ROWS_W; ++j) {
            const int ch = ci0 + (c_first + j) / 3;
#pragma unroll
            for (int hlf = 0; hlf < 2; ++hlf)
                __builtin_amdgcn_raw_ptr_buffer_load_lds(ch < Cin ? in_rs : null_rs, (__attribute__((address_space(3))) void*)(pp + j * Q4_PRW + 64 * hlf), 4,
                                                         m_vo[hlf][j % 3], ch * iHW * 4, 0, 0);
        }
        const unsigned hv = (ci0 + CS <= Cin || ci0 + h_c < Cin) ? h_vo : FAR;
        rh = __uint_as_float(__builtin_amdgcn_raw_buffer_load_b32(ci0 < Cin ? in_rs : null_rs, hv, ci0 * iHW * 4, 0));
    };
    auto store_patch = [&](int buf) __attribute__((always_inline)) {
        float* hd = h_lane ? P + buf * PBUF + p_rows + hj * Q4_PRW + 128 + (lane & 1) : lds + ST_DUMMY + lane;
        *hd = rh;
    };
    unsigned w_vo[DPW];
#pragma unroll
    for (int d = 0; d < DPW; ++d) {
        const int q = wave + NW * d;
        if (q < W4 / 256) {
            const int row = q / (CO_T / 64), co = co0 + (q % (CO_T / 64)) * 64 + lane;
            w_vo[d] = co < Cout ? (unsigned)(row * Cout + co) * 16u : FAR;
        } else if (q < NDMA) {
            constexpr int IPR2 = CO_T / 128 > 0 ? CO_T / 128 : 1;
            const int q2 = q - W4 / 256;
            int row, co;
            if (CO_T >= 128) { row = q2 / IPR2; co = co0 + (q2 % IPR2) * 128 + 2 * lane; }
            else { row = 2 * q2 + (lane >> 5); co = co0 + 2 * (lane & 31); }
            w_vo[d] = co < Cout ? (unsigned)(Cin * 3 * Cout * 4 + (row * Cout + co) * 2) * 4u : FAR;
        } else {
            w_vo[d] = FAR;
        }
    }
    auto dma_weights = [&](int ci0, int buf) __attribute__((always_inline)) {
#pragma unroll
        for (int d = 0; d < DPW; ++d) {
            const int q = wave + NW * d;
            float* dst = q < NDMA ? Wt + buf * WBUF + q * 256 : lds + DMA_DUMMY;
            const int so = q < W4 / 256 ? ci0 * 3 * Cout * 16 : ci0 * 3 * Cout * 8;
            __builtin_amdgcn_raw_ptr_buffer_load_lds(w_rs, (__attribute__((address_space(3))) void*)dst, 16, w_vo[d], so, 0, 0);
        }
    };
    f32x2 xka = {-4.f, -1.f}, xkb = {2.f, -2.f}, xkc = {4.f, -5.f};
    asm volatile("" : "+v"(xka), "+v"(xkb), "+v"(xkc));
    auto kloop = [&](int buf) __attribute__((always_inline)) {
        const float* wa4 = Wt + buf * WBUF + ((lk * KS) * CO_T + wco + li) * 4;
        const float* wa2 = Wt + buf * WBUF + W4 + ((lk * KS) * CO_T + wco + li) * 2;
        const float* pb = P + buf * PBUF + wsg * PSEG + lk * KS * Q4_PRW + 4 * li;
        f32x4 d4[TN], a4[TM];
        f32x2 d2[TN], a2[TM];
        auto reads = [&](int s, f32x4 (&A4)[TM], f32x2 (&A2)[TM], f32x4 (&D4)[TN], f32x2 (&D2)[TN]) __attribute__((always_inline)) {
            const int row = s;
#pragma unroll
            for (int n = 0; n < TN; ++n) {
                D4[n] = *(const f32x4*)(pb + n * PSEG + row * Q4_PRW);
                D2[n] = *(const f32x2*)(pb + n * PSEG + row * Q4_PRW + 4);
            }
#pragma unroll
            for (int i = 0; i < TM; ++i) {
                A4[i] = *(const f32x4*)(wa4 + (row * CO_T + 32 * i) * 4);
                A2[i] = *(const f32x2*)(wa2 + (row * CO_T + 32 * i) * 2);
            }
        };
        constexpr bool PF = NW == 4 && CS != 2;
        reads(0, a4, a2, d4, d2);
#pragma unroll
        for (int s = 0; s < KS; ++s) {
            f32x4 nd4[TN], na4[TM];
            f32x2 nd2[TN], na2[TM];
#pragma unroll
            for (int i = 0; i < TM; ++i) { na4[i] = a4[i]; na2[i] = a2[i]; }
#pragma unroll
            for (int n = 0; n < TN; ++n) { nd4[n] = d4[n]; nd2[n] = d2[n]; }
            if (PF && s + 1 < KS) reads(s + 1, na4, na2, nd4, nd2);
            float vv[TN][6];
#pragma unroll
            for (int n = 0; n < TN; ++n) {
                if (W43_PACKED) {
                    f32x2 v12, v34, v05;
                    w43_input_xform((f32x2){d4[n][0], d4[n][1]}, (f32x2){d4[n][2], d4[n][3]}, d2[n], xka, xkb, xkc, v12, v34, v05);
                    vv[n][0] = v05[0]; vv[n][1] = v12[0]; vv[n][2] = v12[1]; vv[n][3] = v34[0]; vv[n][4] = v34[1]; vv[n][5] = v05[1];
                } else {
                    const float e0 = d4[n][0], e1 = d4[n][1], e2 = d4[n][2], e3 = d4[n][3], e4 = d2[n][0], e5 = d2[n][1];
                    const float ta = __builtin_fmaf(-4.f, e2, e4), tb = __builtin_fmaf(-4.f, e1, e3);
                    const float tc = e4 - e2, td = e3 - e1;
                    vv[n][0] = __builtin_fmaf(4.f, e0, __builtin_fmaf(-5.f, e2, e4));
                    vv[n][1] = ta + tb;
                    vv[n][2] = ta - tb;
                    vv[n][3] = __builtin_fmaf(2.f, td, tc);
                    vv[n][4] = __builtin_fmaf(-2.f, td, tc);
                    vv[n][5] = __builtin_fmaf(4.f, e1, __builtin_fmaf(-5.f, e3, e5));
                }
            }
            __builtin_amdgcn_sched_barrier(0);
#pragma unroll
            for (int x = 0; x < 6; ++x)
#pragma unroll
                for (int i = 0; i < TM; ++i)
#pragma unroll
                    for (int n = 0; n < TN; ++n)
                        acc[i][n][x] = __builtin_amdgcn_mfma_f32_32x32x2f32(x < 4 ? a4[i][x] : a2[i][x - 4], vv[n][x], acc[i][n][x], 0, 0, 0);
            if (PF) {
#pragma unroll
                for (int i = 0; i < TM; ++i) { a4[i] = na4[i]; a2[i] = na2[i]; }
#pragma unroll
                for (int n = 0; n < TN; ++n) { d4[n] = nd4[n]; d2[n] = nd2[n]; }
            } else if (s + 1 < KS) {
                reads(s + 1, a4, a2, d4, d2);
            }
        }
    };

    const int nh = ((Cin + 2 * CS - 1) / (2 * CS)) * 2;
    dma_weights(0, 0);
    load_patch(0, 0);
    store_patch(0);
    for (int h = 0; h < nh; h += 2) {
        __syncthreads();
        if (!(W43_CUT & 1)) { dma_weights((h + 1) * CS, 1); load_patch((h + 1) * CS, 1); }
        kloop(0);
        if (!(W43_CUT & 1)) store_patch(1);
        __syncthreads();
        if (!(W43_CUT & 1)) { dma_weights((h + 2) * CS, 0); load_patch((h + 2) * CS, 0); }
        kloop(1);
        if (!(W43_CUT & 1)) store_patch(0);
    }

#pragma unroll
    for (int n = 0; n < TN; ++n) {
        const WSlot os = wslot((seg0 + n) * Q4_TS + li, geo);
        const int px = 4 * os.k;
        if (!os.valid || os.k >= geo.T || px >= W) continue;
        const int nvalid = min(4, W - px);
        float* obase = out + (long)os.n * Cout * iHW + (long)os.h * W + px;
        const bool vec = nvalid == 4 && ((W & 3) == 0) && ((((uintptr_t)out) & 15) == 0);
#pragma unroll
        for (int i = 0; i < TM; ++i)
#pragma unroll
            for (int r = 0; r < 16; ++r) {
                const int co = co0 + wco + i * 32 + (r & 3) + 8 * (r >> 2) + 4 * lk;
                if (co < Cout) {
                    const float b = bias ? bias[co] : 0.f;
                    const float m0 = acc[i][n][0][r], m1 = acc[i][n][1][r], m2 = acc[i][n][2][r], m3 = acc[i][n][3][r], m4 = acc[i][n][4][r], m5 = acc[i][n][5][r];
                    const float s12 = m1 + m2, d12 = m1 - m2, s34 = m3 + m4, d34 = m3 - m4;
                    f32x4 y;
                    y[0] = ((m0 + s12) + s34) + b;
                    y[1] = __builtin_fmaf(2.f, d34, d12) + b;
                    y[2] = __builtin_fmaf(4.f, s34, s12) + b;
                    y[3] = (__builtin_fmaf(8.f, d34, d12) + m5) + b;
                    float* o = obase + (long)co * iHW;
                    if (vec) *(f32x4*)o = y;
                    else {
#pragma unroll
                        for (int e = 0; e < 4; ++e)
                            if (e < nvalid) o[e] = y[e];
                    }
                }
            }
    }
}
#define VOCR_WINO4_KERNEL(NAME, CO_T, NW, CS, WGS)                                                                                                \
    __global__ __launch_bounds__(64 * NW, WGS) void NAME(const float* __restrict__ in, const float* __restrict__ wpack,                              \
                                                        const float* __restrict__ bias, float* __restrict__ out,                                    \
                                                        const float* __restrict__ zero_page, int N, int Cin, int H, int W, int Cout, WGeom geo,       \
                                                        int co_tiles, const float* __restrict__ wdirect, int n_tail, int first_tail_tile) {          \
        conv3x3_wino4_body<CO_T, NW, CS>(in, wpack, bias, out, zero_page, N, Cin, H, W, Cout, geo, co_tiles, wdirect, n_tail, first_tail_tile);     \
    }
VOCR_WINO4_KERNEL(conv3x3_wino4_kernel_128, 128, 4, 4, 1)
VOCR_WINO4_KERNEL(conv3x3_wino4_kernel_64, 64, 4, 4, 1)
VOCR_WINO4_KERNEL(conv3x3_wino4w8_kernel_128, 128, 8, 4, 1)
VOCR_WINO4_KERNEL(conv3x3_wino4w8_kernel_64, 64, 8, 4, 1)
VOCR_WINO4_KERNEL(conv3x3_wino4x2_kernel_128, 128, 4, 2, 2)
VOCR_WINO4_KERNEL(conv3x3_wino4x2_kernel_64, 64, 4, 2, 2)
#undef VOCR_WINO4_KERNEL


#ifndef W3_CUT
#define W3_CUT 0
#endif
constexpr int G3_DY = 64 * 64;
constexpr int G3_X = 3 * 64 * 64;
constexpr int G3_XE = 6 * 256;
constexpr int G3_XB = G3_X + G3_XE;
constexpr int G3_X0 = 2 * G3_DY;
struct W3Geom { int np, S, slots_img, nseg, adv; };
__device__ __forceinline__ void w3_xform_first(f32x2 g01, f32x2 c01, f32x2 c23, f32x2& a01, f32x2& b01, f32x2& bx) {
    asm("v_pk_add_f32 %0, %3, %3 op_sel:[0,1] op_sel_hi:[0,1] neg_hi:[0,1]\n\t"
        "v_pk_add_f32 %1, %4, %4 op_sel:[0,1] op_sel_hi:[1,0] neg_hi:[0,1]\n\t"
        "v_pk_add_f32 %2, %5, %4 neg_lo:[0,1] neg_hi:[1,0]\n\t"
        "s_nop 1"
        : "=&v"(a01), "=&v"(b01), "=&v"(bx) : "v"(g01), "v"(c01), "v"(c23));
}
__device__ __forceinline__ void w3_xform_second(f32x2 g23, f32x2 c23, f32x2& a23, f32x2& b23) {
    asm("v_pk_add_f32 %0, %2, %2 op_sel:[0,1] op_sel_hi:[0,1] neg_hi:[0,1]\n\t"
        "v_pk_add_f32 %1, %3, %3 op_sel:[0,1] op_sel_hi:[1,0] neg_hi:[0,1]\n\t"
        "s_nop 1"
        : "=&v"(a23), "=&v"(b23) : "v"(g23), "v"(c23));
}

__global__ __launch_bounds__(768) void conv3x3_wgrad_wino3_kernel(const float* __restrict__ x, const float* __restrict__ dy,
                                                                  float* __restrict__ slab, int N, int Cin, int H, int W, int Cout,
                                                                  W3Geom geo, int segs_per_split) {
    __shared__ __attribute__((aligned(256))) float lds[2 * G3_DY + 2 * G3_XB];
    const int tid = threadIdx.x, lane = tid & 63;
    const int wave = __builtin_amdgcn_readfirstlane(tid >> 6);
    const int li = lane & 31, lk = lane >> 5;
    int bx = blockIdx.x, by = blockIdx.y, bz = blockIdx.z;
    if ((gridDim.z & 7) == 0) {
        const int nxy = gridDim.x * gridDim.y;
        const int b = blockIdx.x + gridDim.x * (blockIdx.y + gridDim.y * blockIdx.z);
        const int k = b & 7, slot = b >> 3;
        bz = k + 8 * (slot / nxy);
        const int xy = slot - (slot / nxy) * nxy;
        bx = xy % gridDim.x;
        by = xy / gridDim.x;
    }
    const int ci0 = bx * 64, co0 = by * 64, split = bz;
    const int iHW = H * W;
    const int kh = wave >> 2, wco = ((wave >> 1) & 1) * 32, wci = (wave & 1) * 32;
    const int wq = wave >> 2, wr = wave & 3;

    f32x16 acc[4];
#pragma unroll
    for (int q = 0; q < 4; ++q)
#pragma unroll
        for (int r = 0; r < 16; ++r) acc[q][r] = 0.f;

    const int sbeg = split * segs_per_split;
    const int send = min(geo.nseg, sbeg + segs_per_split);
    const __amdgpu_buffer_rsrc_t dyrs = __builtin_amdgcn_make_buffer_rsrc((void*)dy, 0, (int)((long)N * Cout * iHW * 4), 0x00020000);
    const __amdgpu_buffer_rsrc_t xrs = __builtin_amdgcn_make_buffer_rsrc((void*)x, 0, (int)((long)N * Cin * iHW * 4), 0x00020000);
    constexpr unsigned OOB = 0xFFFFFFF0u;

    struct Slot { int n, h, k; };
    auto decode = [&](int pos) __attribute__((always_inline)) {
        Slot s;
        if (pos < 0) { s.n = 0; s.h = 0; s.k = pos; return s; }
        s.n = pos / geo.slots_img;
        const int r = pos - s.n * geo.slots_img;
        s.h = r / geo.S;
        s.k = r - s.h * geo.S;
        return s;
    };
    auto advance = [&](Slot& s) __attribute__((always_inline)) {
        s.k += 16;
        for (int it = 0; it < geo.adv; ++it) {
            const int c = s.k >= geo.S ? 1 : 0;
            s.k -= c ? geo.S : 0;
            s.h += c;
            const int d = s.h >= H ? 1 : 0;
            s.h -= d ? H : 0;
            s.n += d;
        }
    };
    const int my_ls = ((lane & 15) ^ (lane >> 4)) ^ (4 * wr);
    Slot ms = decode(sbeg * 16 + my_ls);
    const int xt = wq == 1 ? wr : (wq == 2 && wr < 2 ? 4 + wr : -1);
    const int x_which = xt >= 3 ? 1 : 0, x_kh = xt >= 3 ? xt - 3 : xt;
    Slot es = decode(sbeg * 16 + (x_which ? 16 : -1));

    constexpr unsigned FAR = 0x80000000u;
    unsigned d_off[6];
#pragma unroll
    for (int t = 0; t < 6; ++t) {
        const int u = wq + 3 * t;
        if (u < 4) {
            const int co = co0 + 16 * u + 4 * wr + (lane >> 4);
            d_off[t] = co < Cout ? (unsigned)(co * iHW) * 4u : FAR;
        } else if (u < 16) {
            const int i = 4 * (u - 4) + wr, k3 = i >> 4, ci = ci0 + 4 * (i & 15) + (lane >> 4);
            d_off[t] = ci < Cin ? (unsigned)(ci * iHW + (k3 - 1) * W) * 4u : FAR;
        } else {
            const int ci = ci0 + lane;
            d_off[t] = (xt >= 0 && ci < Cin) ? (unsigned)(ci * iHW + (x_kh - 1) * W) * 4u : FAR;
        }
    }
    auto dma = [&](const __amdgpu_buffer_rsrc_t& rs, float* dst, unsigned vo) __attribute__((always_inline)) {
        __builtin_amdgcn_raw_ptr_buffer_load_lds(rs, (__attribute__((address_space(3))) void*)dst, 16, vo, 0, 0, 0);
    };
    auto issue = [&](auto wq_tag, int buf) __attribute__((always_inline)) {
        constexpr int WQ = decltype(wq_tag)::value;
        float* const bdy = lds + buf * G3_DY;
        float* const bx_ = lds + G3_X0 + buf * G3_XB;
        const bool mok = ms.k >= 0 && ms.k < geo.np && ms.n < N;
        const int pix = ms.h * W + 4 * ms.k;
        const unsigned dyb = mok ? (unsigned)(ms.n * Cout * iHW + pix) * 4u : FAR;
        const unsigned xmid = mok ? (unsigned)(ms.n * Cin * iHW + pix) * 4u : FAR;
        const unsigned xb3[3] = {ms.h >= 1 ? xmid : FAR, xmid, ms.h + 1 < H ? xmid : FAR};
#pragma unroll
        for (int t = 0; t < 6; ++t) {
            const int u = WQ + 3 * t;
            if (u < 4) dma(dyrs, bdy + (4 * u + wr) * 256, dyb + d_off[t]);
            else if (u < 16) dma(xrs, bx_ + (4 * (u - 4) + wr) * 256, xb3[(u - 4) >> 2] + d_off[t]);
            else if (xt >= 0) {
                const int row = es.h + x_kh - 1;
                const bool eok = es.k >= 0 && es.k < geo.np && es.n < N && row >= 0 && row < H;
                dma(xrs, bx_ + G3_X + xt * 256, (eok ? (unsigned)(es.n * Cin * iHW + es.h * W + 4 * es.k) * 4u : FAR) + d_off[t]);
            }
        }
    };
    auto patch = [&](auto wq_tag, int buf) __attribute__((always_inline)) {
        constexpr int WQ = decltype(wq_tag)::value;
        if ((W & 3) == 0) return;
        float* const bdy = lds + buf * G3_DY;
        float* const bx_ = lds + G3_X0 + buf * G3_XB;
        const int nv = W - 4 * (geo.np - 1);
        if (ms.k == geo.np - 1) {
#pragma unroll
            for (int t = 0; t < 6; ++t) {
                const int u = WQ + 3 * t;
                if (u < 16) {
                    float* o = (u < 4 ? bdy + (4 * u + wr) * 256 : bx_ + (4 * (u - 4) + wr) * 256) + lane * 4;
#pragma unroll
                    for (int e = 1; e < 4; ++e)
                        if (e >= nv) o[e] = 0.f;
                }
            }
        }
        if (xt >= 0 && es.k == geo.np - 1) {
// ... 349 lines not shown
                w4_xform_b<!PLUS>((f32x2){cur.ca[0], cur.ca[1]}, (f32x2){cur.ca[2], cur.ca[3]}, (f32x2){cur.cb[0], cur.cb[1]},
                                  (f32x2){cur.cb[2], cur.cb[3]}, c01, c23, b0, bx2, b1);
                const float p = PLUS ? cur.pa + cur.pb : cur.pa - cur.pb;
                const float n = PLUS ? cur.na + cur.nb : cur.na - cur.nb;
                const float e0 = p - c01[1], e1 = n - c23[0];
#pragma unroll
                for (int s = 0; s < 2; ++s) {
                    f32x2 g01, g23, a0, a1;
                    if (V == 0 || V == 3) {
                        const f32x4 g = V == 0 ? cur.g0[s] : cur.g1[s];
                        g01 = (f32x2){g[0], g[1]}; g23 = (f32x2){g[2], g[3]};
                        w4_xform_a(g01, g23, a0, a1);
                    } else {
                        w4_xform_a2<V == 2>((f32x2){cur.g0[s][0], cur.g0[s][1]}, (f32x2){cur.g0[s][2], cur.g0[s][3]},
                                            (f32x2){cur.g1[s][0], cur.g1[s][1]}, (f32x2){cur.g1[s][2], cur.g1[s][3]}, g01, g23, a0, a1);
                    }
                    acc[s][0] = __builtin_amdgcn_mfma_f32_32x32x2f32(g01[0], e0, acc[s][0], 0, 0, 0);
                    acc[s][1] = __builtin_amdgcn_mfma_f32_32x32x2f32(a0[0], b0[0], acc[s][1], 0, 0, 0);
                    acc[s][2] = __builtin_amdgcn_mfma_f32_32x32x2f32(a0[1], b0[1], acc[s][2], 0, 0, 0);
                    acc[s][3] = __builtin_amdgcn_mfma_f32_32x32x2f32(g01[1], bx2[0], acc[s][3], 0, 0, 0);
                    acc[s][0] = __builtin_amdgcn_mfma_f32_32x32x2f32(g23[0], bx2[1], acc[s][0], 0, 0, 0);
                    acc[s][1] = __builtin_amdgcn_mfma_f32_32x32x2f32(a1[0], b1[0], acc[s][1], 0, 0, 0);
                    acc[s][2] = __builtin_amdgcn_mfma_f32_32x32x2f32(a1[1], b1[1], acc[s][2], 0, 0, 0);
                    acc[s][3] = __builtin_amdgcn_mfma_f32_32x32x2f32(g23[1], e1, acc[s][3], 0, 0, 0);
                }
                cur = nxt;
            }
            if (more) {
                __builtin_amdgcn_s_waitcnt(0x0F70);
                patch(decltype(cur_tag)::value ^ 1, last_piece);
            }
            __syncthreads();
        };
        for (int q = 0; q < nloc; q += 2) {
            segment(std::integral_constant<int, 0>{}, q, q + 1 < nloc);
            if (q + 1 < nloc) segment(std::integral_constant<int, 1>{}, q + 1, q + 2 < nloc);
        }
    };

    fill(0, 64);
    __syncthreads();
    if (nloc > 0) {
        const Entry e = entry(0);
        issue(0, e);
        __builtin_amdgcn_s_waitcnt(0x0F70);
        patch(0, e.t1.z);
    }
    __syncthreads();
    if (v == 0) run(std::integral_constant<int, 0>{});
    else if (v == 1) run(std::integral_constant<int, 1>{});
    else if (v == 2) run(std::integral_constant<int, 2>{});
    else run(std::integral_constant<int, 3>{});
    const long plane = (long)Cout * Cin;
    const float sc = (v == 1 || v == 2) ? 0.5f : 1.0f;
#pragma unroll
    for (int s = 0; s < 2; ++s)
#pragma unroll
        for (int r = 0; r < 16; ++r) {
            const int co = co0 + 32 * s + (r & 3) + 8 * (r >> 2) + 4 * lk;
            const int ci = ci0 + cB;
            if (co < Cout && ci < Cin) {
                const float m0 = sc * acc[s][0][r], m1 = 0.5f * sc * acc[s][1][r], m2 = 0.5f * sc * acc[s][2][r], m3 = sc * acc[s][3][r];
                float* o = slab + ((long)split * 12 + v * 3) * plane + (long)co * Cin + ci;
                o[0] = (m0 + m1) + m2;
                o[plane] = m1 - m2;
                o[2 * plane] = (m1 + m2) + m3;
            }
        }
}

template <int G>
__global__ __launch_bounds__(64 * G) void wgrad_reduce2d_kernel(const float* __restrict__ slab, float* __restrict__ dw, int Cout, int Cin,
                                                                int splits) {
    __shared__ f32x4 red[G][4][64];
    const long plane = (long)Cout * Cin;
    const long per_kw = plane / 4;
    const int lane = threadIdx.x & 63, g = threadIdx.x >> 6;
    const long o = (long)blockIdx.x * 64 + lane;
    const bool ok = o < 3 * per_kw;
    const int kw = ok ? (int)(o / per_kw) : 0;
    const long r4 = ok ? o - (long)kw * per_kw : 0;
    f32x4 s[4];
#pragma unroll
    for (int vv = 0; vv < 4; ++vv) s[vv] = (f32x4){0.f, 0.f, 0.f, 0.f};
    if (ok)
        for (int sp = g; sp < splits; sp += G)
#pragma unroll
            for (int vv = 0; vv < 4; ++vv) s[vv] += *(const f32x4*)(slab + ((long)sp * 12 + vv * 3 + kw) * plane + r4 * 4);
#pragma unroll
    for (int vv = 0; vv < 4; ++vv) red[g][vv][lane] = s[vv];
    __syncthreads();
    if (g == 0 && ok) {
        f32x4 t[4];
#pragma unroll
        for (int vv = 0; vv < 4; ++vv) {
            f32x4 u[G];
#pragma unroll
            for (int i = 0; i < G; ++i) u[i] = red[i][vv][lane];
#pragma unroll
            for (int w = 1; w < G; w *= 2)
#pragma unroll
                for (int i = 0; i + w < G; i += 2 * w) u[i] += u[i + w];
            t[vv] = u[0];
        }
        const f32x4 s12 = t[1] + t[2];
        const f32x4 k0 = t[0] + s12, k1 = t[1] - t[2], k2 = s12 + t[3];
#pragma unroll
        for (int e = 0; e < 4; ++e) {
            float* d = dw + (r4 * 4 + e) * 9 + kw;
            d[0] = k0[e];
            d[3] = k1[e];
            d[6] = k2[e];
        }
    }
}


const float* wino_zero_page_ptr() {
    static const float* zp[64] = {nullptr};
    int dev = 0;
    if (hipGetDevice(&dev) != hipSuccess || dev < 0 || dev >= 64) return nullptr;
    if (!zp[dev]) {
        void* p = nullptr;
        if (hipGetSymbolAddress(&p, HIP_SYMBOL(g_wino_zero_page)) != hipSuccess) return nullptr;
        zp[dev] = (const float*)p;
    }
    return zp[dev];
}

}

extern "C" int vocr_conv3x3_wino_supported(int cin, int cout) { return cin >= 1 && cout % 4 == 0 ? 1 : 0; }

extern "C" size_t vocr_conv3x3_wino_pack_floats(int cout, int cin) { return (size_t)cout * cin * (wino4_for(cout) ? 27 : 21); }

extern "C" int vocr_conv3x3_wino_pack_weights(const float* w, float* wpack_fwd, float* wpack_dgrad, int cout, int cin, void* stream) {
    VOCR_CHECK_ARG(w && (wpack_fwd || wpack_dgrad), "vocr_conv3x3_wino_pack_weights: null pointer");
    VOCR_CHECK_ARG(cout > 0 && cin > 0, "vocr_conv3x3_wino_pack_weights: bad shape");
    const int total = cout * cin * 3;
    const bool f4f = wpack_fwd && wino4_for(cout), f4d = wpack_dgrad && wino4_for(cin);
    hipStream_t s = (hipStream_t)stream;
    if (f4f || f4d) wino4_pack_kernel<<<vocr_cdiv(total, 256), 256, 0, s>>>(w, f4f ? wpack_fwd : nullptr, f4d ? wpack_dgrad : nullptr, cout, cin);
    if ((wpack_fwd && !f4f) || (wpack_dgrad && !f4d))
        wino_pack_kernel<<<vocr_cdiv(total, 256), 256, 0, s>>>(w, f4f ? nullptr : wpack_fwd, f4d ? nullptr : wpack_dgrad, cout, cin, wino_pack_x4());
    VOCR_CHECK_LAUNCH("vocr_conv3x3_wino_pack_weights");
    int rc = VOCR_OK;
    if (wpack_fwd) rc = vocr_conv3x3_pack_weights(w, wpack_fwd + (size_t)cout * cin * (f4f ? 18 : 12), nullptr, cout, cin, stream);
    if (rc == VOCR_OK && wpack_dgrad) rc = vocr_conv3x3_pack_weights(w, nullptr, wpack_dgrad + (size_t)cout * cin * (f4d ? 18 : 12), cout, cin, stream);
    return rc;
}

namespace {
enum WinoKind { WK_F23_64 = 1, WK_F23_128, WK_W4_64, WK_W4_128, WK_W8_64, WK_W8_128, WK_X2_64, WK_X2_128, WK_R3_64, WK_R3_128 };
struct WinoPlan { int kind, n_tail, n_main; WGeom geo; };

int wino_cu_count() {
    int ncu = 256, dev = 0;
    hipDeviceProp_t prop;
    if (hipGetDevice(&dev) == hipSuccess && hipGetDeviceProperties(&prop, dev) == hipSuccess && prop.multiProcessorCount > 0) ncu = prop.multiProcessorCount;
    return ncu;
}

WinoPlan wino_plan_of(int n, int cin, int h, int w, int cout, int ncu) {
    WinoPlan p = {0, 0, 0, {}};
    if (n <= 0 || cin <= 0 || h <= 0 || w <= 0 || cout <= 0 || cout % 4 != 0) return p;
    const long big = (long)n * (cin > cout ? cin : cout) * h * w;
    if (big >= (1l << 31)) return p;
    const bool f43 = wino4_for(cout);
    if (f43 && big >= (1l << 29)) return p;
    WGeom& geo = p.geo;
    geo.T = vocr_cdiv(w, f43 ? 4 : 2);
    geo.S = geo.T + 1;
    geo.slots_img = h * geo.S;
    geo.nslot = n * geo.slots_img;
    geo.nseg = vocr_cdiv(geo.nslot, TS);
    static const int tail_mode = VOCR_EXPERIMENT_INT("VOCR_CONV_TAIL", 1);
    if (f43) {
        const int t8 = vocr_cdiv(geo.nseg, 4) * vocr_cdiv(cout, 128);
        const bool x2 = wino4_mode() != 6 && wino4_mode() != 3 && wino4_mode() != 4 &&
                        (wino4_mode() == 5 || (cout > 64 ? vocr_cdiv(geo.nseg, 2) * vocr_cdiv(cout, 128) : vocr_cdiv(geo.nseg, 4)) >= 2 * ncu);
        const int nw = (wino4_mode() == 3 || x2) ? 4 : wino4_mode() == 4 ? 8 : (t8 >= ncu ? 8 : 4);
        const int tiles4 = cout > 64 ? vocr_cdiv(geo.nseg, nw / 2) * vocr_cdiv(cout, 128) : vocr_cdiv(geo.nseg, nw);
        const int slots4 = x2 ? 2 * ncu : ncu;
        const int rem4 = tiles4 % slots4;
        const bool cut4 = tail_mode == 1 && tiles4 > slots4 && rem4 > 0 && rem4 <= slots4 / 2;
        p.n_main = cut4 ? tiles4 - rem4 : tiles4;
        p.n_tail = cut4 ? rem4 * 8 * nw : 0;
        p.kind = x2 ? (cout > 64 ? WK_X2_128 : WK_X2_64) : nw == 8 ? (cout > 64 ? WK_W8_128 : WK_W8_64) : (cout > 64 ? WK_W4_128 : WK_W4_64);
        return p;
    }
    const bool f23 = wino2_mode() && big < (1l << 29);
    p.kind = cout > 64 ? (f23 ? WK_F23_128 : WK_R3_128) : (f23 ? WK_F23_64 : WK_R3_64);
    const int co_t = cout > 64 ? 128 : 64, nseg_t = cout > 64 ? 2 : 4, co_tiles = cout > 64 ? vocr_cdiv(cout, 128) : 1;
    const int tiles = vocr_cdiv(geo.nseg, nseg_t) * co_tiles, rem = tiles % ncu;
    const bool cut = tail_mode == 1 && tiles > ncu && rem > 0 && (rem <= ncu / 4 || (rem <= ncu / 2 && cin >= 128));
    p.n_main = cut ? tiles - rem : tiles;
    p.n_tail = cut ? rem * (co_t / 32) * 2 * nseg_t : 0;
    return p;
}
}

extern "C" int vocr_conv3x3_wino_plan(int n, int cin, int h, int w, int cout) {
    const WinoPlan p = wino_plan_of(n, cin, h, w, cout, wino_cu_count());
    return p.kind == 0 ? 0 : p.kind + (p.n_tail > 0 ? 16 : 0);
}

extern "C" int vocr_conv3x3_wino_fwd(const float* x, const float* wpack, const float* bias, float* y, int n, int cin, int h,
                                     int w, int cout, void* stream) {
    VOCR_CHECK_ARG(x && wpack && y, "vocr_conv3x3_wino_fwd: null pointer");
    VOCR_CHECK_ARG(n > 0 && cin > 0 && h > 0 && w > 0 && cout > 0, "vocr_conv3x3_wino_fwd: bad shape");
    VOCR_CHECK_ARG(cout % 4 == 0 && ((((uintptr_t)wpack) & 15) == 0), "vocr_conv3x3_wino_fwd: needs Cout %% 4 == 0 and a 16-byte aligned pack");
    VOCR_CHECK_ARG((long)n * (cin > cout ? cin : cout) * h * w < (1l << 31), "vocr_conv3x3_wino_fwd: tensor exceeds 2^31 elements");
    const bool f43 = wino4_for(cout);
    VOCR_CHECK_ARG(!f43 || (long)n * (cin > cout ? cin : cout) * h * w < (1l << 29), "vocr_conv3x3_wino_fwd: the F(4,3) kernel needs tensors below 2^29 elements");
    const WinoPlan p = wino_plan_of(n, cin, h, w, cout, wino_cu_count());
    VOCR_CHECK_ARG(p.kind != 0, "vocr_conv3x3_wino_fwd: no kernel for this shape");
    const WGeom geo = p.geo;
    const float* zp = wino_zero_page_ptr();
    VOCR_CHECK_ARG(zp != nullptr, "vocr_conv3x3_wino_fwd: no device zero page");
    hipStream_t s = (hipStream_t)stream;
    const float* wdirect = wpack + (size_t)cin * (f43 ? 18 : 12) * cout;
    const dim3 grid(p.n_tail + p.n_main);
    const int ct = vocr_cdiv(cout, 128);
    switch (p.kind) {
        case WK_X2_128: conv3x3_wino4x2_kernel_128<<<grid, 256, 0, s>>>(x, wpack, bias, y, zp, n, cin, h, w, cout, geo, ct, wdirect, p.n_tail, p.n_main); break;
        case WK_W8_128: conv3x3_wino4w8_kernel_128<<<grid, 512, 0, s>>>(x, wpack, bias, y, zp, n, cin, h, w, cout, geo, ct, wdirect, p.n_tail, p.n_main); break;
        case WK_W4_128: conv3x3_wino4_kernel_128<<<grid, 256, 0, s>>>(x, wpack, bias, y, zp, n, cin, h, w, cout, geo, ct, wdirect, p.n_tail, p.n_main); break;
        case WK_X2_64: conv3x3_wino4x2_kernel_64<<<grid, 256, 0, s>>>(x, wpack, bias, y, zp, n, cin, h, w, cout, geo, 1, wdirect, p.n_tail, p.n_main); break;
        case WK_W8_64: conv3x3_wino4w8_kernel_64<<<grid, 512, 0, s>>>(x, wpack, bias, y, zp, n, cin, h, w, cout, geo, 1, wdirect, p.n_tail, p.n_main); break;
        case WK_W4_64: conv3x3_wino4_kernel_64<<<grid, 256, 0, s>>>(x, wpack, bias, y, zp, n, cin, h, w, cout, geo, 1, wdirect, p.n_tail, p.n_main); break;
        case WK_F23_128: conv3x3_wino2_kernel_128<<<grid, 256, 0, s>>>(x, wpack, bias, y, zp, n, cin, h, w, cout, geo, ct, wdirect, p.n_tail, p.n_main); break;
        case WK_F23_64: conv3x3_wino2_kernel_64<<<grid, 256, 0, s>>>(x, wpack, bias, y, zp, n, cin, h, w, cout, geo, 1, wdirect, p.n_tail, p.n_main); break;
        case WK_R3_128: conv3x3_wino_kernel<128><<<grid, 256, 0, s>>>(x, wpack, bias, y, zp, n, cin, h, w, cout, geo, ct, wdirect, p.n_tail, p.n_main); break;
        default: conv3x3_wino_kernel<64><<<grid, 256, 0, s>>>(x, wpack, bias, y, zp, n, cin, h, w, cout, geo, 1, wdirect, p.n_tail, p.n_main); break;
    }
    VOCR_CHECK_LAUNCH("vocr_conv3x3_wino_fwd");
    return VOCR_OK;
}

void vocr_internal_wgrad_reduce(const float* slab, float* dw, int cout, int cin, int splits, hipStream_t s);

namespace {
int wgrad_wino3_splits(int n, int cin, int h, int w, int cout, W3Geom* geo, int* segs_per_split) {
    geo->np = vocr_cdiv(w, 4);
    geo->S = geo->np + 1;
    geo->slots_img = h * geo->S;
    const long nslot = (long)n * geo->slots_img;
    geo->nseg = (int)((nslot + 15) / 16);
    geo->adv = vocr_cdiv(16, geo->S);
    const int tiles = vocr_cdiv(cin, 64) * vocr_cdiv(cout, 64);
    long s = (256 + tiles - 1) / tiles;
    if (s > geo->nseg) s = geo->nseg;
    if (s < 1) s = 1;
    const int sps = (int)((geo->nseg + s - 1) / s);
    *segs_per_split = sps;
    return (geo->nseg + sps - 1) / sps;
}
int wgrad_wino2d_splits(int n, int cin, int h, int w, int cout, W3Geom* geo, int* segs_per_split) {
    geo->np = vocr_cdiv(w, 4);
    geo->S = geo->np + 1;
    geo->slots_img = vocr_cdiv(h, 2) * geo->S;
    const long nslot = (long)n * geo->slots_img;
    geo->nseg = (int)((nslot + 7) / 8);
    geo->adv = vocr_cdiv(8, geo->S);
    const int tiles = vocr_cdiv(cin, 64) * vocr_cdiv(cout, 64);
    long s = (256 + tiles - 1) / tiles;
    if (s > geo->nseg) s = geo->nseg;
    if (s < 1) s = 1;
    const int sps = (int)((geo->nseg + s - 1) / s);
    *segs_per_split = sps;
    return (geo->nseg + sps - 1) / sps;
}
int wgrad_wino_mode() {
    static const int m = VOCR_EXPERIMENT_INT("VOCR_WGRAD_WINO_DMA", 3);
    return m == 2 ? 2 : 3;
}
}

extern "C" size_t vocr_conv3x3_wgrad_wino_workspace_bytes(int n, int cin, int h, int w, int cout) {
    if (n <= 0 || cin <= 0 || h <= 0 || w <= 0 || cout <= 0) return 0;
    int sps;
    W3Geom g3;
    if (wgrad_wino_mode() == 3 && (cout * cin) % 4 == 0) return (size_t)wgrad_wino2d_splits(n, cin, h, w, cout, &g3, &sps) * 12 * cout * cin * sizeof(float);
    return (size_t)wgrad_wino3_splits(n, cin, h, w, cout, &g3, &sps) * 9 * cout * cin * sizeof(float);
}

extern "C" int vocr_conv3x3_wgrad_wino(const float* x, const float* dy, float* dw, void* workspace, int n, int cin, int h, int w,
                                       int cout, void* stream) {
    VOCR_CHECK_ARG(x && dy && dw && workspace, "vocr_conv3x3_wgrad_wino: null pointer");
    VOCR_CHECK_ARG(n > 0 && cin >= 4 && h > 0 && w > 0 && cout > 0, "vocr_conv3x3_wgrad_wino: bad shape (needs cin >= 4)");
    VOCR_CHECK_ARG((long)n * (cin > cout ? cin : cout) * h * w < (1l << 29), "vocr_conv3x3_wgrad_wino: tensor exceeds 2^29 elements (32-bit byte offsets)");
    hipStream_t s = (hipStream_t)stream;
    int sps, splits;
    if (wgrad_wino_mode() == 3 && (cout * cin) % 4 == 0) {
        W3Geom g4;
        splits = wgrad_wino2d_splits(n, cin, h, w, cout, &g4, &sps);
        dim3 grid(vocr_cdiv(cin, 64), vocr_cdiv(cout, 64), splits);
        conv3x3_wgrad_wino2d_kernel<<<grid, 512, 0, s>>>(x, dy, (float*)workspace, n, cin, h, w, cout, g4, sps);
        VOCR_CHECK_LAUNCH("vocr_conv3x3_wgrad_wino(row pairs)");
        const long total4 = 3l * cout * cin / 4;
        const int wgs = (int)((total4 + 63) / 64);
        if (wgs < 64 && splits >= 64) wgrad_reduce2d_kernel<16><<<wgs, 1024, 0, s>>>((const float*)workspace, dw, cout, cin, splits);
        else wgrad_reduce2d_kernel<4><<<wgs, 256, 0, s>>>((const float*)workspace, dw, cout, cin, splits);
        VOCR_CHECK_LAUNCH("vocr_conv3x3_wgrad_wino(row pairs, reduce)");
        return VOCR_OK;
    }
    W3Geom g3;
    splits = wgrad_wino3_splits(n, cin, h, w, cout, &g3, &sps);
    dim3 grid(vocr_cdiv(cin, 64), vocr_cdiv(cout, 64), splits);
    conv3x3_wgrad_wino3_kernel<<<grid, 768, 0, s>>>(x, dy, (float*)workspace, n, cin, h, w, cout, g3, sps);
    VOCR_CHECK_LAUNCH("vocr_conv3x3_wgrad_wino");
    vocr_internal_wgrad_reduce((const float*)workspace, dw, cout, cin, splits, s);
    VOCR_CHECK_LAUNCH("vocr_conv3x3_wgrad_wino(reduce)");
    return VOCR_OK;
}
```

vistaocr_amd/csrc/vocr_common.h:

```cpp
#pragma once
#include <hip/hip_runtime.h>
#include <stdint.h>
#include <stdio.h>
#include "../../include/vocr.h"

typedef float f32x4 __attribute__((ext_vector_type(4)));
typedef float f32x16 __attribute__((ext_vector_type(16)));

#define VOCR_WAVE 64

#ifdef VOCR_EXPERIMENTS
#include <stdlib.h>
#define VOCR_EXPERIMENT_INT(name, dflt) (getenv(name) ? atoi(getenv(name)) : (dflt))
#else
#define VOCR_EXPERIMENT_INT(name, dflt) (dflt)
#endif

void vocr_set_error(const char* fmt, ...);

#define VOCR_CHECK_ARG(cond, ...)                 \
    do {                                          \
        if (!(cond)) {                            \
            vocr_set_error(__VA_ARGS__);          \
            return VOCR_EINVAL;                   \
        }                                         \
    } while (0)

#define VOCR_CHECK_LAUNCH(name)                                                       \
    do {                                                                              \
        hipError_t e__ = hipGetLastError();                                           \
        if (e__ != hipSuccess) {                                                      \
            vocr_set_error("%s: launch failed: %s", name, hipGetErrorString(e__));    \
            return VOCR_ELAUNCH;                                                      \
        }                                                                             \
    } while (0)

static inline int vocr_cdiv(long a, long b) { return (int)((a + b - 1) / b); }

struct VocrPerDevice {
    bool set[64];
};
int vocr_allow_dynamic_lds(const void* const* kernels, int n, int bytes, VocrPerDevice* done, const char* who);

__device__ __forceinline__ float wave_sum(float v) {
#pragma unroll
    for (int o = 32; o > 0; o >>= 1) v += __shfl_xor(v, o, 64);
    return v;
}
__device__ __forceinline__ double wave_sum_d(double v) {
#pragma unroll
    for (int o = 32; o > 0; o >>= 1) v += __shfl_xor(v, o, 64);
    return v;
}
__device__ __forceinline__ float wave_max(float v) {
#pragma unroll
    for (int o = 32; o > 0; o >>= 1) v = fmaxf(v, __shfl_xor(v, o, 64));
    return v;
}
```

vistaocr_amd/ops.py:

```python
import math

import torch

from . import _lib
from ._lib import call, prof_range


def _stream():
    return torch.cuda.current_stream().cuda_stream


def _ranged(name):
    def deco(fn):
        if not _lib.ROCTX:
            return fn

        def wrapped(*a, **k):
            with prof_range(name):
                return fn(*a, **k)
        wrapped.__name__ = fn.__name__
        wrapped.__doc__ = fn.__doc__
        return wrapped
    return deco

# ... 60 lines not shown
def join_side_stream(device=None):
    if not torch.cuda.is_available():
        return
    idx = torch.cuda.current_device() if device is None else torch.device(device).index
    st = _SIDE.get(idx)
    if st is not None and st["pending"]:
        torch.cuda.current_stream(idx).wait_stream(st["stream"])
        st["pending"] = False


_HEALTH = {}


def health(device):
    idx = torch.device(device).index
    if idx is None:
        idx = torch.cuda.current_device()
    h = _HEALTH.get(idx)
    if h is None:
        h = _HEALTH[idx] = torch.zeros(2, dtype=torch.int32, device=torch.device("cuda", idx))
    return h


def reset_health(device=None):
    if device is None:
        device = torch.device("cuda", torch.cuda.current_device())
    health(device).zero_()


def check_health(values, device=None):
    bad0, bad1 = int(values[0]) != 0, int(values[1]) != 0
    if (bad0 or bad1) and device is not None:
        reset_health(device)
    if bad0:
        raise RuntimeError("vistaocr_amd: a hand-off inside a persistent LSTM sweep timed out (its output is NaN-poisoned); "
                           "is another persistent sweep running on this GPU?  VOCR_LSTM_SWEEP=step selects per-step launches")
    if bad1:
        raise RuntimeError("vistaocr_amd: a NaN gradient reached the optimiser (the reference's clamp_ would propagate it too)")


def check_health_sync(device):
    check_health(health(device).cpu().tolist(), device)


def _sinks(params):
    owner = None
    out = []
    for p in params:
        o = getattr(p, "_vocr_sink_owner", None)
        g = p.grad
        if o is None or (owner is not None and o is not owner) or g is None or not g.is_cuda or not g.is_contiguous() \
                or g.dtype != torch.float32:
            return None
        owner = o
        out.append(g)
    if owner is None or not owner.owns_grads(params):
        return None
    owner.note_direct_write(params)
    return out


def _fire(hooks, name):
    if hooks:
        for fn in hooks.get(name, ()):
            fn()


def _ws(nbytes, device):
    return torch.empty((max(int(nbytes), 16) + 3) // 4, dtype=torch.float32, device=device)


class ForwardPrep(object):
    def __init__(self):
        self.packs = {}
        self.lstm = {}
        self.xpack = {}
        self.x6w = {}
        self.event = None
        self.pack_events = {}
        self._waited = False

    def wait(self):
        if not self._waited and self.event is not None:
            torch.cuda.current_stream().wait_event(self.event)
            self._waited = True

    def wait_pack(self, key):
        ev = self.pack_events.get(key)
        if ev is not None and not self._waited:
            torch.cuda.current_stream().wait_event(ev)


def lstm_bias_sum(b_ih_f, b_hh_f, b_ih_r, b_hh_r):
    H4 = b_ih_f.numel()
    bsum = torch.empty(2, H4, dtype=torch.float32, device=b_ih_f.device)
    call("vocr_add", _p(b_ih_f), _p(b_hh_f), _p(bsum[0]), H4, _stream())
    call("vocr_add", _p(b_ih_r), _p(b_hh_r), _p(bsum[1]), H4, _stream())
    return bsum


def lstm_xproj_pack(w_ih_f, w_ih_r):
    h = w_ih_f.shape[0] // 4
    wpack = torch.empty(_lib.load().vocr_lstm_xproj_pack_bytes(h) // 4, dtype=torch.float32, device=w_ih_f.device)
    call("vocr_lstm_xproj_pack", _p(w_ih_f), _p(w_ih_r), _p(wpack), h, _stream())
    return wpack


def x6_weight_planes(w_ih_f, w_ih_r, with_transpose):
    g4, din = w_ih_f.shape
    wk = x6_planes(w_ih_f, 2 * g4, din, True, din, x2=w_ih_r, seg=g4, axis=1)
    wt = x6_planes(w_ih_f, din, 2 * g4, False, din, x2=w_ih_r, seg=g4, axis=0) if with_transpose else None
    return wk, wt


def forward_prep(conv_weights, lstm_layers, with_transposes, f16=False, follow_layers=(), x6_layers=()):
    if not _SIDE_ENABLED or _exp("VOCR_FWD_PREP", "1") != "1":
        return None
    prep = ForwardPrep()
    main = torch.cuda.current_stream()
    side = side_stream()
    side.wait_stream(main)
    made = []
    with torch.cuda.stream(side):
        for w in conv_weights:
            pk = conv3x3_pack_f16(w) if f16 else conv3x3_pack(w)
            prep.packs[w.data_ptr()] = pk
            made.extend(pk)
            ev = torch.cuda.Event()
            ev.record(side)
            prep.pack_events[w.data_ptr()] = ev
        for (w_hh_f, b_ih_f, b_hh_f, w_hh_r, b_ih_r, b_hh_r) in lstm_layers:
            H4 = b_ih_f.numel()
            bsum = torch.empty(2, H4, dtype=torch.float32, device=b_ih_f.device)
            call("vocr_add", _p(b_ih_f), _p(b_hh_f), _p(bsum[0]), H4, _stream())
            call("vocr_add", _p(b_ih_r), _p(b_hh_r), _p(bsum[1]), H4, _stream())
            wt = (transpose2d(w_hh_f), transpose2d(w_hh_r)) if with_transposes else (None, None)
            prep.lstm[w_hh_f.data_ptr()] = (bsum, wt[0], wt[1])
            made.extend(t for t in (bsum,) + wt if t is not None)
        for (w_ih_f, w_ih_r) in x6_layers:
            if w_ih_f.shape[1] >= 512:
                prep.x6w[w_ih_f.data_ptr()] = x6_weight_planes(w_ih_f, w_ih_r, with_transposes)
                made.extend(t for t in prep.x6w[w_ih_f.data_ptr()] if t is not None)
        for (w_ih_f, w_ih_r) in follow_layers:
            prep.xpack[w_ih_f.data_ptr()] = lstm_xproj_pack(w_ih_f, w_ih_r)
            made.append(prep.xpack[w_ih_f.data_ptr()])
        prep.event = torch.cuda.Event()
        prep.event.record(side)
    for t in made:
        t.record_stream(main)
    return prep


_BN_FUSED_FINAL = _exp("VOCR_BN_FUSED_FINAL", "1") == "1"
_WINO = _exp("VOCR_CONV_WINO", "1") == "1"
_WINO_WGRAD = _exp("VOCR_WGRAD_WINO", "1") == "1"


_WINO_MIN_CIN = int(_exp("VOCR_CONV_WINO_MIN_CIN", "1"))


def _wino_ok(cin, cout):
    return _WINO and cin >= _WINO_MIN_CIN and cout % 4 == 0


def conv3x3_pack(weight):
    cout, cin = weight.shape[0], weight.shape[1]
    dev = weight.device
    wf, wd = _wino_ok(cin, cout), _wino_ok(cout, cin)
    lib = _lib.load()
    rows_f = lib.vocr_conv3x3_wino_pack_floats(cout, cin) // (cout * cin)
    rows_d = lib.vocr_conv3x3_wino_pack_floats(cin, cout) // (cout * cin)
    pf = torch.empty(cin * (rows_f if wf else 9), cout, dtype=torch.float32, device=dev)
    pd = torch.empty(cout * (rows_d if wd else 9), cin, dtype=torch.float32, device=dev)
    if wf or wd:
        call("vocr_conv3x3_wino_pack_weights", _p(weight), _p(pf) if wf else None, _p(pd) if wd else None, cout, cin, _stream())
    if not (wf and wd):
        call("vocr_conv3x3_pack_weights", _p(weight), None if wf else _p(pf), None if wd else _p(pd), cout, cin, _stream())
    return pf, pd


def conv3x3_pack_f16(weight):
    cout, cin = weight.shape[0], weight.shape[1]
    lib = _lib.load()
    pf = torch.empty(lib.vocr_conv3x3_f16_pack_bytes(cout, cin, 0) // 2, dtype=torch.float16, device=weight.device)
    pd = torch.empty(lib.vocr_conv3x3_f16_pack_bytes(cout, cin, 1) // 2, dtype=torch.float16, device=weight.device)
    call("vocr_conv3x3_f16_pack_weights", _p(weight), _p(pf), _p(pd), cout, cin, _stream())
    return pf, pd


def f16_layouts(x, want_nhwc=True, want_nchwp=False):
    n, c, h, w = x.shape
    nhwc = torch.empty(n, c // 16, h, w, 16, dtype=torch.float16, device=x.device) if want_nhwc else None
    nchwp = torch.empty(n, c, h, _lib.load().vocr_f16_padded_row(w), dtype=torch.float16, device=x.device) if want_nchwp else None
    call("vocr_f32_to_f16_layouts", _p(x), _p(nhwc), _p(nchwp), n, c, h, w, _stream())
    return nhwc, nchwp


def h16_takes(n, cin, h, w, cout):
    return bool(_lib.load().vocr_conv3x3_h16_supported(cin, cout)) and n * h <= 65535 and n * h * w * max(cin, cout) * 2 < 2 ** 31


def conv3x3_forward_f16(x, wpack16, bias, cout, x_nhwc=None):
    n, cin, h, w = x.shape
    y = torch.empty(n, cout, h, w, dtype=torch.float32, device=x.device)
    if h16_takes(n, cin, h, w, cout):
        if x_nhwc is None:
            x_nhwc = f16_layouts(x)[0]
        call("vocr_conv3x3_h16_fwd", _p(x_nhwc), _p(wpack16), _p(bias), _p(y), n, cin, h, w, cout, _stream())
    else:
        call("vocr_conv3x3_f16_fwd", _p(x), _p(wpack16), _p(bias), _p(y), n, cin, h, w, cout, _stream())
    return y


def wgrad_f16_layouts_ok(cin, cout):
    return bool(_lib.load().vocr_conv3x3_wgrad_h16_supported(cin, cout))


def conv3x3_forward(x, wpack, bias, cout):
    n, cin, h, w = x.shape
    y = torch.empty(n, cout, h, w, dtype=torch.float32, device=x.device)
    lib = _lib.load()
    rows = wpack.shape[0] if wpack.dim() == 2 else -1
    wino_rows = lib.vocr_conv3x3_wino_pack_floats(cout, cin) // (cout * cin) * cin if lib.vocr_conv3x3_wino_supported(cin, cout) else -2
    if wpack.dim() != 2 or wpack.shape[1] != cout or rows not in (9 * cin, wino_rows):
        raise ValueError("conv3x3_forward: weight pack %s does not fit cin=%d cout=%d (expected %d or %d rows)"
                         % (tuple(wpack.shape), cin, cout, 9 * cin, wino_rows))
    if rows != 9 * cin and n * max(cin, cout) * h * w >= (1 << 29):
        wpack = wpack[rows - 9 * cin:]
        rows = 9 * cin
    fn = "vocr_conv3x3_wino_fwd" if rows != 9 * cin else "vocr_conv3x3_fwd"
    call(fn, _p(x), _p(wpack), _p(bias), _p(y), n, cin, h, w, cout, _stream())
    return y


def conv3x3_c1_forward(x, weight, bias, f16=False):
    n, _, h, w = x.shape
    cout = weight.shape[0]
    y = torch.empty(n, cout, h, w, dtype=torch.float32, device=x.device)
    call("vocr_conv3x3_c1_fwd", _p(x), _p(weight), _p(bias), _p(y), n, h, w, cout, int(bool(f16)), _stream())
    return y


def conv3x3_c1_wgrad_takes(cin, cout):
    return cin == 1 and cout < 32


def conv3x3_wgrad(x, dy, out=None, f16=False, x16p=None, dy16p=None, dbias_out=None):
    n, cin, h, w = x.shape
    cout = dy.shape[1]
    lib = _lib.load()
    dw = out if out is not None else torch.empty(cout, cin, 3, 3, dtype=torch.float32, device=x.device)
    if conv3x3_c1_wgrad_takes(cin, cout):
        ws = _ws(lib.vocr_conv3x3_c1_wgrad_workspace_bytes(n, h, cout), x.device)
        call("vocr_conv3x3_c1_wgrad", _p(x), _p(dy), _p(dw), _p(dbias_out), _p(ws), n, h, w, cout, _stream())
        return dw
    if f16 and x16p is not None and dy16p is not None:
        ws = _ws(lib.vocr_conv3x3_wgrad_h16_workspace_bytes(n, cin, h, w, cout), x.device)
        call("vocr_conv3x3_wgrad_h16", _p(x16p), _p(dy16p), _p(dw), _p(ws), n, cin, h, w, cout, _stream())
        return dw
    if _WINO_WGRAD and cin >= 4 and n * max(cin, cout) * h * w < (1 << 29):
        ws = _ws(lib.vocr_conv3x3_wgrad_wino_workspace_bytes(n, cin, h, w, cout), x.device)
        call("vocr_conv3x3_wgrad_wino", _p(x), _p(dy), _p(dw), _p(ws), n, cin, h, w, cout, _stream())
        return dw
    ws = _ws(lib.vocr_conv3x3_wgrad_workspace_bytes(n, cin, h, w, cout), x.device)
    call("vocr_conv3x3_wgrad_f16" if f16 else "vocr_conv3x3_wgrad", _p(x), _p(dy), _p(dw), _p(ws), n, cin, h, w, cout, _stream())
    return dw


def channel_sum(x, out=None):
    n, c, h, w = x.shape
    out = out if out is not None else torch.empty(c, dtype=torch.float32, device=x.device)
    nb = _lib.load().vocr_channel_sum_workspace_bytes(n, c, h * w)
    ws = _ws(nb, x.device) if nb else None
    call("vocr_channel_sum", _p(x), _p(out), n, c, h * w, _p(ws), _stream())
    return out


class ConvBnReluFn(torch.autograd.Function):

    @staticmethod
    def forward(ctx, x, weight, bias, gamma, beta, running_mean, running_var, training, eps, momentum, f16=False,
                pool_samples=None, pool_oh=0, pool_ow=0, num_batches_tracked=None, prep=None):
        _need_gpu(x, weight, bias, gamma, beta, running_mean, running_var)
        x = _f32c(x)
        n, cin, h, w = x.shape
        cout = weight.shape[0]
        lib = _lib.load()
        ctx.f16 = bool(f16)
        x16p = None
        if cin == 1 and not ctx.needs_input_grad[0]:
            pf = pd = None
            y = conv3x3_c1_forward(x, weight, bias, ctx.f16)
        elif ctx.f16:
            if prep is not None and weight.data_ptr() in prep.packs:
                prep.wait_pack(weight.data_ptr())
                pf, pd = prep.packs[weight.data_ptr()]
            else:
                pf, pd = conv3x3_pack_f16(weight)
            x_nhwc = None
            if h16_takes(n, cin, h, w, cout):
                x_nhwc, x16p = f16_layouts(x, True, bool(training) and wgrad_f16_layouts_ok(cin, cout))
            y = conv3x3_forward_f16(x, pf, bias, cout, x_nhwc)
        else:
            if prep is not None and weight.data_ptr() in prep.packs:
                prep.wait_pack(weight.data_ptr())
                pf, pd = prep.packs[weight.data_ptr()]
            else:
                pf, pd = conv3x3_pack(weight)
            y = conv3x3_forward(x, pf, bias, cout)
        mean = torch.empty(cout, dtype=torch.float32, device=x.device)
        invstd = torch.empty(cout, dtype=torch.float32, device=x.device)
        xhat_sum = None
        fused_final = training and _BN_FUSED_FINAL
        ws = None
        if training:
            ws = _ws(lib.vocr_bn_workspace_bytes(n, cout, h * w), x.device)
            xhat_sum = torch.empty(cout, dtype=torch.float32, device=x.device)
            if not fused_final:
                call("vocr_bn_train_stats", _p(y), n, cout, h * w, eps, momentum, _p(mean), _p(invstd), _p(running_mean),
                     _p(running_var), _p(num_batches_tracked), _p(xhat_sum), _p(ws), _stream())
        else:
            call("vocr_bn_eval_stats", _p(running_mean), _p(running_var), cout, eps, _p(mean), _p(invstd), _stream())
        ctx.pool = None
        idx = samples = None
        if pool_samples is not None:
            samples = _f32c(pool_samples)
            if tuple(samples.shape) != (n, cout, 2):
                raise RuntimeError("fractional pool samples must have shape (N, C, 2)")
            out = torch.empty(n, cout, pool_oh, pool_ow, dtype=torch.float32, device=x.device)
            idx = torch.empty(n, cout, pool_oh, pool_ow, dtype=torch.int32, device=x.device)
            if fused_final:
                call("vocr_bn_train_relu_fracpool2x2_fwd", _p(y), _p(gamma), _p(beta), _p(samples), _p(out), _p(idx), n, cout, h, w, pool_oh, pool_ow,
                     eps, momentum, _p(mean), _p(invstd), _p(running_mean), _p(running_var), _p(num_batches_tracked), _p(xhat_sum), _p(ws), _stream())
            else:
                call("vocr_bn_relu_fracpool2x2_fwd", _p(y), _p(mean), _p(invstd), _p(gamma), _p(beta), _p(samples), _p(out), _p(idx),
                     n, cout, h, w, pool_oh, pool_ow, _stream())
            ctx.pool = (pool_oh, pool_ow)
        else:
            out = torch.empty_like(y)
            if fused_final:
                call("vocr_bn_train_relu_apply", _p(y), _p(gamma), _p(beta), _p(out), n, cout, h * w, eps, momentum, _p(mean), _p(invstd),
                     _p(running_mean), _p(running_var), _p(num_batches_tracked), _p(xhat_sum), _p(ws), _stream())
            else:
                call("vocr_bn_relu_apply", _p(y), _p(mean), _p(invstd), _p(gamma), _p(beta), _p(out), n, cout, h * w, _stream())
        ctx.training = training
        ctx.prefs = (weight, bias, gamma, beta)
        ctx.save_for_backward(x, y, mean, invstd, gamma, beta, pd, idx, samples, xhat_sum, x16p)
        return out

    @staticmethod
    @_ranged("bwd.conv_bn_relu")
    def backward(ctx, da):
        if not ctx.training:
            raise RuntimeError("vistaocr_amd: backward through eval-mode BatchNorm is not part of the reference path")
        x, y, mean, invstd, gamma, beta, pd, idx, samples, xhat_sum, x16p = ctx.saved_tensors
        da = _f32c(da)
        n, cin, h, w = x.shape
        cout = y.shape[1]
        lib = _lib.load()
        fused_pool_bwd = False
        if ctx.pool is not None:
            oh, ow = ctx.pool
            fused_pool_bwd = bool(lib.vocr_bn_relu_fracpool2x2_bwd_supported(h, w, oh, ow)) and _exp("VOCR_POOL_BWD_FUSED", "1") == "1"
            if not fused_pool_bwd:
                dfull = torch.empty(n, cout, h, w, dtype=torch.float32, device=da.device)
                call("vocr_fracpool2x2_bwd", _p(da), _p(idx), _p(dfull), n, cout, h, w, oh, ow, _stream())
                da = dfull
        dy = torch.empty_like(y)
        sinks = _sinks(ctx.prefs)
        if sinks is not None:
            dw, dbias, dgamma, dbeta = sinks
        else:
            dw = None
            dgamma = torch.empty_like(gamma)
            dbeta = torch.empty_like(beta)
            dbias = torch.empty(cout, dtype=torch.float32, device=x.device)
        ws = _ws(lib.vocr_bn_workspace_bytes(n, cout, h * w), x.device)
        if fused_pool_bwd:
            call("vocr_bn_relu_fracpool2x2_bwd", _p(da), _p(idx), _p(samples), _p(y), _p(mean), _p(invstd), _p(gamma), _p(beta),
                 _p(xhat_sum), _p(dy), _p(dgamma), _p(dbeta), _p(dbias), n, cout, h, w, oh, ow, _p(ws), _stream())
        else:
            call("vocr_bn_relu_bwd", _p(da), _p(y), _p(mean), _p(invstd), _p(gamma), _p(beta), _p(xhat_sum), _p(dy), _p(dgamma),
                 _p(dbeta), _p(dbias), n, cout, h * w, _p(ws), _stream())
        dy_nhwc = dy16p = None
        if ctx.f16:
            want_nhwc = bool(ctx.needs_input_grad[0]) and h16_takes(dy.shape[0], cout, dy.shape[2], dy.shape[3], cin)
            if want_nhwc or x16p is not None:
                dy_nhwc, dy16p = f16_layouts(dy, want_nhwc, x16p is not None)
        if sinks is not None and _SIDE_ENABLED and ctx.needs_input_grad[0] and _exp("VOCR_CONV_OVERLAP", "1") == "1":
            side = side_stream()
            side.wait_stream(torch.cuda.current_stream())
            for t_ in (x, dy, x16p, dy16p):
                if t_ is not None:
                    t_.record_stream(side)
            with torch.cuda.stream(side):
                conv3x3_wgrad(x, dy, out=dw, f16=ctx.f16, x16p=x16p, dy16p=dy16p)
            mark_side_pending()
        else:
            dw = conv3x3_wgrad(x, dy, out=dw, f16=ctx.f16, x16p=x16p, dy16p=dy16p)
        dx = None
        if ctx.needs_input_grad[0]:
            dx = conv3x3_forward_f16(dy, pd, None, cin, dy_nhwc) if ctx.f16 else conv3x3_forward(dy, pd, None, cin)
        else:
            join_side_stream()
        if sinks is not None:
            return (dx,) + (None,) * 15
        return (dx, dw, dbias, dgamma, dbeta) + (None,) * 11


class ConvReluPoolFn(torch.autograd.Function):

    @staticmethod
    def forward(ctx, x, weight, bias, f16=False):
        _need_gpu(x, weight, bias)
        x = _f32c(x)
        n, cin, h, w = x.shape
        cout = weight.shape[0]
        ctx.f16 = bool(f16)
        if cin == 1 and not ctx.needs_input_grad[0]:
            pf = pd = None
            y = conv3x3_c1_forward(x, weight, bias, ctx.f16)
        elif ctx.f16:
            pf, pd = conv3x3_pack_f16(weight)
            y = conv3x3_forward_f16(x, pf, bias, cout)
        else:
            pf, pd = conv3x3_pack(weight)
            y = conv3x3_forward(x, pf, bias, cout)
        oh, ow = h // 2, w // 2
        out = torch.empty(n, cout, oh, ow, dtype=torch.float32, device=x.device)
        idx = torch.empty(n, cout, oh, ow, dtype=torch.int32, device=x.device)
        call("vocr_relu_maxpool2_fwd", _p(y), _p(out), _p(idx), n, cout, h, w, _stream())
        ctx.save_for_backward(x, out, idx, pd)
        ctx.prefs = (weight, bias)
        ctx.hw = (h, w)
        return out

    @staticmethod
    @_ranged("bwd.rapid_ds")
    def backward(ctx, dout):
        x, out, idx, pd = ctx.saved_tensors
        dout = _f32c(dout)
        n, cin, _, _ = x.shape
        cout = out.shape[1]
        h, w = ctx.hw
        dy = torch.zeros(n, cout, h, w, dtype=torch.float32, device=x.device)
        call("vocr_relu_maxpool2_bwd", _p(dout), _p(out), _p(idx), _p(dy), n, cout, h, w, _stream())
        sinks = _sinks(ctx.prefs)
        if conv3x3_c1_wgrad_takes(cin, cout):
            dbias = sinks[1] if sinks else torch.empty(cout, dtype=torch.float32, device=x.device)
            dw = conv3x3_wgrad(x, dy, out=sinks[0] if sinks else None, f16=ctx.f16, dbias_out=dbias)
        else:
            dbias = channel_sum(dy, out=sinks[1] if sinks else None)
            dw = conv3x3_wgrad(x, dy, out=sinks[0] if sinks else None, f16=ctx.f16)
        dx = None
        if ctx.needs_input_grad[0]:
            dx = conv3x3_forward_f16(dy, pd, None, cin) if ctx.f16 else conv3x3_forward(dy, pd, None, cin)
        else:
            join_side_stream()
        if sinks is not None:
            return dx, None, None, None
        return dx, dw, dbias, None


class FracPoolFn(torch.autograd.Function):

    @staticmethod
    def forward(ctx, x, samples, oh, ow):
        _need_gpu(x, samples)
        x = _f32c(x)
# ... 944 lines not shown
```

Measured before the change: 2289 line-images/sec.

## Fuse BatchNorm sum/sumsq partials into Winograd conv forward epilogue

The Winograd F(4,3) conv forward kernels now optionally compute per-channel sum and sum-of-squares of their output in double precision, reduced through LDS and shuffles, and write per-tile partials to an armed workspace. The fused BN train kernels then fold these partials with a small kernel instead of re-reading the whole conv output to compute statistics. This removes one full read pass over the activation per conv+BN layer for large layers, at the cost of extra epilogue work, __syncthreads inside the conv kernel, and a thread-local handshake between host calls.

```diff
diff --git a/include/vocr.h b/include/vocr.h
--- a/include/vocr.h
+++ b/include/vocr.h
@@ -75,6 +75,9 @@
                                        int32_t* idx, int n, int c, int h, int w, int oh, int ow, float eps, float momentum,
                                        float* mean, float* invstd, float* running_mean, float* running_var,
                                        int64_t* num_batches_tracked, float* xhat_sum, void* workspace, void* stream);
+int vocr_conv3x3_wino_bn_slots(int n, int cin, int h, int w, int cout);
+size_t vocr_bn_epilogue_workspace_bytes(int c, int slots);
+int vocr_bn_epilogue_arm(void* workspace, int slots);
 int vocr_bn_relu_bwd(const float* da, const float* y, const float* mean, const float* invstd,
                      const float* gamma, const float* beta, const float* xhat_sum, float* dy, float* dgamma, float* dbeta,
                      float* dconv_bias, int n, int c, int hw, void* workspace, void* stream);
diff --git a/vistaocr_amd/_lib.py b/vistaocr_amd/_lib.py
--- a/vistaocr_amd/_lib.py
+++ b/vistaocr_amd/_lib.py
@@ -47,6 +47,9 @@
     "vocr_bn_relu_apply": (I, [P, P, P, P, P, P, I, I, I, P]),
     "vocr_bn_train_relu_apply": (I, [P, P, P, P, I, I, I, F, F, P, P, P, P, P, P, P, P]),
     "vocr_bn_train_relu_fracpool2x2_fwd": (I, [P, P, P, P, P, P, I, I, I, I, I, I, F, F, P, P, P, P, P, P, P, P]),
+    "vocr_conv3x3_wino_bn_slots": (I, [I, I, I, I, I]),
+    "vocr_bn_epilogue_workspace_bytes": (Z, [I, I]),
+    "vocr_bn_epilogue_arm": (I, [P, I]),
     "vocr_bn_relu_bwd": (I, [P, P, P, P, P, P, P, P, P, P, P, I, I, I, P, P]),
     "vocr_bn_relu_fracpool2x2_bwd_supported": (I, [I, I, I, I]),
     "vocr_bn_relu_fracpool2x2_bwd": (I, [P] * 13 + [I] * 6 + [P, P]),
diff --git a/vistaocr_amd/csrc/bn_pool.hip b/vistaocr_amd/csrc/bn_pool.hip
--- a/vistaocr_amd/csrc/bn_pool.hip
+++ b/vistaocr_amd/csrc/bn_pool.hip
@@ -121,6 +121,22 @@
     __syncthreads();
     s = stage[2 * BN_MAX_CHUNKS];
     q = stage[2 * BN_MAX_CHUNKS + 1];
+}
+
+__global__ __launch_bounds__(256) void bn_fold_partials_kernel(const double* __restrict__ part, double* __restrict__ folded, int nslot) {
+    __shared__ double red[8];
+    const int c = blockIdx.x;
+    const double* p = part + (long)c * nslot * 2;
+    double a = 0.0, b = 0.0;
+    for (int j = threadIdx.x; j < nslot; j += 256) {
+        a += p[2 * j];
+        b += p[2 * j + 1];
+    }
+    block_reduce2(a, b, red);
+    if (threadIdx.x == 0) {
+        folded[2 * c] = a;
+        folded[2 * c + 1] = b;
+    }
 }
 
 __device__ __forceinline__ void bn_train_stats_of(double s, double q, long count, float eps, float momentum, int c, bool writer,
@@ -649,6 +665,45 @@
     return (size_t)c * bn_nchunk((long)n * hw) * 2 * sizeof(double);
 }
 
+VocrBnEpilogue* vocr_internal_bn_epilogue() {
+    static thread_local VocrBnEpilogue ep = {nullptr, 0, 0};
+    return &ep;
+}
+
+extern "C" size_t vocr_bn_epilogue_workspace_bytes(int c, int slots) {
+    if (c <= 0 || slots <= 0) return 0;
+    return (size_t)c * ((size_t)slots + 1) * 2 * sizeof(double);
+}
+
+extern "C" int vocr_bn_epilogue_arm(void* workspace, int slots) {
+    VocrBnEpilogue* ep = vocr_internal_bn_epilogue();
+    ep->part = nullptr;
+    ep->slots = 0;
+    ep->delivered = 0;
+    if (!workspace && slots == 0) return VOCR_OK;
+    VOCR_CHECK_ARG(workspace && slots > 0 && (((uintptr_t)workspace) & 15) == 0, "vocr_bn_epilogue_arm: needs a 16-byte aligned workspace and slots > 0");
+    ep->part = (double*)workspace;
+    ep->slots = slots;
+    return VOCR_OK;
+}
+
+namespace {
+bool bn_take_epilogue(void* workspace, int c, hipStream_t s, const double** part, int* nslot) {
+    VocrBnEpilogue* ep = vocr_internal_bn_epilogue();
+    const bool got = ep->delivered && ep->part == (double*)workspace && ep->slots > 0;
+    const int slots = ep->slots;
+    ep->part = nullptr;
+    ep->slots = 0;
+    ep->delivered = 0;
+    if (!got) return false;
+    double* folded = (double*)workspace + (size_t)c * slots * 2;
+    bn_fold_partials_kernel<<<c, 256, 0, s>>>((const double*)workspace, folded, slots);
+    *part = folded;
+    *nslot = 1;
+    return true;
+}
+}
+
 extern "C" int vocr_bn_train_stats(const float* y, int n, int c, int hw, float eps, float momentum, float* mean,
                                    float* invstd, float* running_mean, float* running_var, int64_t* num_batches_tracked,
                                    float* xhat_sum, void* workspace, void* stream) {
@@ -716,9 +771,11 @@
     VOCR_CHECK_ARG((long)n * c <= 65535, "vocr_bn_train_relu_apply: n*c > 65535 planes");
     hipStream_t s = (hipStream_t)stream;
     int nchunk = 0;
-    bn_launch_partial(y, n, c, hw, workspace, s, &nchunk);
+    const double* part = (const double*)workspace;
+    const bool from_conv = bn_take_epilogue(workspace, c, s, &part, &nchunk);
+    if (!from_conv) bn_launch_partial(y, n, c, hw, workspace, s, &nchunk);
     VOCR_CHECK_LAUNCH("vocr_bn_train_relu_apply(partial)");
-    const BnFusedStats fs = {(const double*)workspace, nchunk, (long)n * hw, eps, momentum, mean, invstd, running_mean, running_var, xhat_sum,
+    const BnFusedStats fs = {part, nchunk, (long)n * hw, eps, momentum, mean, invstd, running_mean, running_var, xhat_sum,
                              (long long*)num_batches_tracked};
     const int V = vec_width(hw, y, out);
     const dim3 grid = plane_grid((long)n * c, hw / V);
@@ -819,9 +876,11 @@
                    "vocr_bn_train_relu_fracpool2x2_fwd: bad shape h=%d w=%d oh=%d ow=%d", h, w, oh, ow);
     hipStream_t s = (hipStream_t)stream;
     int nchunk = 0;
-    bn_launch_partial(y, n, c, h * w, workspace, s, &nchunk);
+    const double* part = (const double*)workspace;
+    const bool from_conv = bn_take_epilogue(workspace, c, s, &part, &nchunk);
+    if (!from_conv) bn_launch_partial(y, n, c, h * w, workspace, s, &nchunk);
     VOCR_CHECK_LAUNCH("vocr_bn_train_relu_fracpool2x2_fwd(partial)");
-    const BnFusedStats fs = {(const double*)workspace, nchunk, (long)n * h * w, eps, momentum, mean, invstd, running_mean, running_var, xhat_sum,
+    const BnFusedStats fs = {part, nchunk, (long)n * h * w, eps, momentum, mean, invstd, running_mean, running_var, xhat_sum,
                              (long long*)num_batches_tracked};
     const float alpha_h = oh > 1 ? (float)(h - 2) / (float)(oh - 1) : 0.f;
     const float alpha_w = ow > 1 ? (float)(w - 2) / (float)(ow - 1) : 0.f;
diff --git a/vistaocr_amd/csrc/conv_tail.h b/vistaocr_amd/csrc/conv_tail.h
--- a/vistaocr_amd/csrc/conv_tail.h
+++ b/vistaocr_amd/csrc/conv_tail.h
@@ -5,16 +5,28 @@
 
 struct SegInfo { long base; int n; int h; int w0; int valid; int rows; int pw; int ow; };
 
+__device__ __forceinline__ double tail_shfl_xor_d(double v, int m) {
+    const int lo = __shfl_xor(__double2loint(v), m, 64), hi = __shfl_xor(__double2hiint(v), m, 64);
+    return __hiloint2double(hi, lo);
+}
+
 template <int TAIL_WAVES>
 __device__ __forceinline__ void conv3x3_tail_piece_px(float* __restrict__ red_, int pn, int ph, int pwc, bool pix_ok, bool live, int co_base,
                                                       const float* __restrict__ in, const float* __restrict__ wpack, const float* __restrict__ bias,
-                                                      float* __restrict__ out, const float* __restrict__ zero_page, int Cin, int H, int W, int Cout) {
+                                                      float* __restrict__ out, const float* __restrict__ zero_page, int Cin, int H, int W, int Cout,
+                                                      double* __restrict__ bn_part = nullptr, int bn_slots = 0, int bn_slot = 0) {
     float (*red)[16][64] = (float (*)[16][64])red_;
     const int tid = threadIdx.x, lane = tid & 63;
     const int wave = __builtin_amdgcn_readfirstlane(tid >> 6);
     const int li = lane & 31, lk = lane >> 5;
     (void)li;
-    if (!live || co_base >= Cout) return;
+    if (!live || co_base >= Cout) {
+        if (bn_part && tid < 32 && co_base + tid < Cout) {
+            bn_part[((long)(co_base + tid) * bn_slots + bn_slot) * 2] = 0.0;
+            bn_part[((long)(co_base + tid) * bn_slots + bn_slot) * 2 + 1] = 0.0;
+        }
+        return;
+    }
     const long HW = (long)H * W;
     int toff[9];
     float tm[9];
@@ -68,8 +80,21 @@
 #pragma unroll
         for (int w8 = 0; w8 < TAIL_WAVES; ++w8) sum += red[w8][r][lane];
         const int oc = co_base + (r & 3) + 8 * (r >> 2) + 4 * lk;
-        if (pix_ok && oc < Cout)
-            out[(long)pn * Cout * HW + (long)oc * HW + (long)ph * W + pwc] = sum + (bias ? bias[oc] : 0.f);
+        const bool ok = pix_ok && oc < Cout;
+        const float val = sum + ((bias && oc < Cout) ? bias[oc] : 0.f);
+        if (ok) out[(long)pn * Cout * HW + (long)oc * HW + (long)ph * W + pwc] = val;
+        if (bn_part) {
+            double s = ok ? (double)val : 0.0, q = s * s;
+#pragma unroll
+            for (int o = 16; o > 0; o >>= 1) {
+                s += tail_shfl_xor_d(s, o);
+                q += tail_shfl_xor_d(q, o);
+            }
+            if ((lane & 31) == 0 && oc < Cout) {
+                bn_part[((long)oc * bn_slots + bn_slot) * 2] = s;
+                bn_part[((long)oc * bn_slots + bn_slot) * 2 + 1] = q;
+            }
+        }
     }
 }
 
diff --git a/vistaocr_amd/csrc/conv_wino.hip b/vistaocr_amd/csrc/conv_wino.hip
--- a/vistaocr_amd/csrc/conv_wino.hip
+++ b/vistaocr_amd/csrc/conv_wino.hip
@@ -499,7 +499,8 @@
 template <int CO_T, int NW, int CS>
 __device__ __forceinline__ void conv3x3_wino4_body(const float* __restrict__ in, const float* __restrict__ wpack, const float* __restrict__ bias,
                                                    float* __restrict__ out, const float* __restrict__ zero_page, int N, int Cin, int H, int W, int Cout,
-                                                   WGeom geo, int co_tiles, const float* __restrict__ wdirect, int n_tail, int first_tail_tile) {
+                                                   WGeom geo, int co_tiles, const float* __restrict__ wdirect, int n_tail, int first_tail_tile,
+                                                   double* __restrict__ bn_part) {
     constexpr int TM = 2, TN = 1;
     constexpr int WAVES_CO = CO_T / 64;
     constexpr int NSEG = NW / WAVES_CO;
@@ -524,8 +525,10 @@
         const int pli = threadIdx.x & 31;
         const WSlot ps = wslot(q0 + (pli >> 2), geo);
         const int pcol = 4 * ps.k + (pli & 3);
+        const int bn_ptcut = first_tail_tile / co_tiles, bn_slots = bn_ptcut + ((geo.nseg + NSEG - 1) / NSEG - bn_ptcut) * (4 * NSEG);
         conv3x3_tail_piece_px<NW>(lds, ps.n, ps.h, pcol, ps.valid && ps.k < geo.T && pcol < W, q0 < geo.nslot,
-                                 (vt % co_tiles) * CO_T + (sub % COSUB) * 32, in, wdirect, bias, out, zero_page, Cin, H, W, Cout);
+                                 (vt % co_tiles) * CO_T + (sub % COSUB) * 32, in, wdirect, bias, out, zero_page, Cin, H, W, Cout, bn_part, bn_slots,
+                                 bn_ptcut + (vt / co_tiles - bn_ptcut) * (4 * NSEG) + pb);
         return;
     }
     const int tid = threadIdx.x, lane = tid & 63;
@@ -705,36 +708,106 @@
         if (!(W43_CUT & 1)) store_patch(0);
     }
 
+    constexpr int BN_TR = 16 * 33 * 2;
+    static_assert((NW * (BN_TR + 128)) * 2 <= 2 * WBUF + 2 * PBUF, "the BatchNorm reduction must fit the main loop's LDS");
+    double* const bn_tr = (double*)lds + wave * BN_TR;
+    double* const bn_ws = (double*)lds + NW * BN_TR + wave * 128;
+    if (bn_part) {
+        asm volatile("s_waitcnt vmcnt(0)" ::: "memory");
+        __syncthreads();
+    }
 #pragma unroll
     for (int n = 0; n < TN; ++n) {
         const WSlot os = wslot((seg0 + n) * Q4_TS + li, geo);
         const int px = 4 * os.k;
-        if (!os.valid || os.k >= geo.T || px >= W) continue;
+        const bool live = os.valid && os.k < geo.T && px < W;
+        if (!bn_part && !live) continue;
         const int nvalid = min(4, W - px);
         float* obase = out + (long)os.n * Cout * iHW + (long)os.h * W + px;
         const bool vec = nvalid == 4 && ((W & 3) == 0) && ((((uintptr_t)out) & 15) == 0);
 #pragma unroll
         for (int i = 0; i < TM; ++i)
 #pragma unroll
-            for (int r = 0; r < 16; ++r) {
-                const int co = co0 + wco + i * 32 + (r & 3) + 8 * (r >> 2) + 4 * lk;
-                if (co < Cout) {
-                    const float b = bias ? bias[co] : 0.f;
-                    const float m0 = acc[i][n][0][r], m1 = acc[i][n][1][r], m2 = acc[i][n][2][r], m3 = acc[i][n][3][r], m4 = acc[i][n][4][r], m5 = acc[i][n][5][r];
-                    const float s12 = m1 + m2, d12 = m1 - m2, s34 = m3 + m4, d34 = m3 - m4;
-                    f32x4 y;
-                    y[0] = ((m0 + s12) + s34) + b;
-                    y[1] = __builtin_fmaf(2.f, d34, d12) + b;
-                    y[2] = __builtin_fmaf(4.f, s34, s12) + b;
-                    y[3] = (__builtin_fmaf(8.f, d34, d12) + m5) + b;
-                    float* o = obase + (long)co * iHW;
-                    if (vec) *(f32x4*)o = y;
-                    else {
-#pragma unroll
-                        for (int e = 0; e < 4; ++e)
-                            if (e < nvalid) o[e] = y[e];
+            for (int hf = 0; hf < 2; ++hf) {
+#pragma unroll
+                for (int rr = 0; rr < 8; ++rr) {
+                    const int r = hf * 8 + rr;
+                    const int co = co0 + wco + i * 32 + (r & 3) + 8 * (r >> 2) + 4 * lk;
+                    double bs = 0.0, bq = 0.0;
+                    if (live && co < Cout) {
+                        const float b = bias ? bias[co] : 0.f;
+                        const float m0 = acc[i][n][0][r], m1 = acc[i][n][1][r], m2 = acc[i][n][2][r], m3 = acc[i][n][3][r], m4 = acc[i][n][4][r], m5 = acc[i][n][5][r];
+                        const float s12 = m1 + m2, d12 = m1 - m2, s34 = m3 + m4, d34 = m3 - m4;
+                        f32x4 y;
+                        y[0] = ((m0 + s12) + s34) + b;
+                        y[1] = __builtin_fmaf(2.f, d34, d12) + b;
+                        y[2] = __builtin_fmaf(4.f, s34, s12) + b;
+                        y[3] = (__builtin_fmaf(8.f, d34, d12) + m5) + b;
+                        float* o = obase + (long)co * iHW;
+                        if (vec) *(f32x4*)o = y;
+                        else {
+#pragma unroll
+                            for (int e = 0; e < 4; ++e)
+                                if (e < nvalid) o[e] = y[e];
+                        }
+                        if (bn_part) {
+#pragma unroll
+                            for (int e = 0; e < 4; ++e)
+                                if (e < nvalid) {
+                                    const double yd = (double)y[e];
+                                    bs += yd;
+                                    bq = __builtin_fma(yd, yd, bq);
+                                }
+                        }
+                    }
+                    if (bn_part) {
+                        double* t = bn_tr + ((rr * 2 + lk) * 33 + li) * 2;
+                        t[0] = bs;
+                        t[1] = bq;
                     }
                 }
+                if (bn_part) {
+                    __syncthreads();
+                    const int cl = lane & 15, g = lane >> 4;
+                    const double* t = bn_tr + (cl * 33 + 8 * g) * 2;
+                    double cs = 0.0, cq = 0.0;
+#pragma unroll
+                    for (int j = 0; j < 8; ++j) {
+                        cs += t[2 * j];
+                        cq += t[2 * j + 1];
+                    }
+                    cs += __shfl_xor(cs, 16, 64);
+                    cq += __shfl_xor(cq, 16, 64);
+                    cs += __shfl_xor(cs, 32, 64);
+                    cq += __shfl_xor(cq, 32, 64);
+                    if (lane < 16) {
+                        const int r = hf * 8 + (cl >> 1);
+                        const int ch = i * 32 + (r & 3) + 8 * (r >> 2) + 4 * (cl & 1);
+                        bn_ws[2 * ch] = cs;
+                        bn_ws[2 * ch + 1] = cq;
+                    }
+                    __syncthreads();
+                }
+            }
+    }
+    if (bn_part && tid < CO_T && co0 + tid < Cout) {
+        const int pt = v / co_tiles;
+        const int bn_ptcut = first_tail_tile / co_tiles, bn_slots = bn_ptcut + ((geo.nseg + NSEG - 1) / NSEG - bn_ptcut) * (4 * NSEG);
+        const double* wsum = (const double*)lds + NW * BN_TR + ((tid >> 6) * NSEG) * 128 + (tid & 63) * 2;
+        double cs = 0.0, cq = 0.0;
+#pragma unroll
+        for (int sg = 0; sg < NSEG; ++sg) {
+            cs += wsum[sg * 128];
+            cq += wsum[sg * 128 + 1];
+        }
+        const int slot = pt < bn_ptcut ? pt : bn_ptcut + (pt - bn_ptcut) * (4 * NSEG);
+        double* dst = bn_part + ((long)(co0 + tid) * bn_slots + slot) * 2;
+        dst[0] = cs;
+        dst[1] = cq;
+        if (pt >= bn_ptcut)
+            for (int j = 1; j < 4 * NSEG; ++j) {
+                dst[2 * j] = 0.0;
+                dst[2 * j + 1] = 0.0;
             }
     }
 }
@@ -742,8 +815,10 @@
     __global__ __launch_bounds__(64 * NW, WGS) void NAME(const float* __restrict__ in, const float* __restrict__ wpack,                              \
                                                         const float* __restrict__ bias, float* __restrict__ out,                                    \
                                                         const float* __restrict__ zero_page, int N, int Cin, int H, int W, int Cout, WGeom geo,       \
-                                                        int co_tiles, const float* __restrict__ wdirect, int n_tail, int first_tail_tile) {          \
-        conv3x3_wino4_body<CO_T, NW, CS>(in, wpack, bias, out, zero_page, N, Cin, H, W, Cout, geo, co_tiles, wdirect, n_tail, first_tail_tile);     \
+                                                        int co_tiles, const float* __restrict__ wdirect, int n_tail, int first_tail_tile,            \
+                                                        double* __restrict__ bn_part) {                                                             \
+        conv3x3_wino4_body<CO_T, NW, CS>(in, wpack, bias, out, zero_page, N, Cin, H, W, Cout, geo, co_tiles, wdirect, n_tail, first_tail_tile,      \
+                                         bn_part);                                                                                                 \
     }
 VOCR_WINO4_KERNEL(conv3x3_wino4_kernel_128, 128, 4, 4, 1)
 VOCR_WINO4_KERNEL(conv3x3_wino4_kernel_64, 64, 4, 4, 1)
@@ -1399,7 +1474,7 @@
 
 namespace {
 enum WinoKind { WK_F23_64 = 1, WK_F23_128, WK_W4_64, WK_W4_128, WK_W8_64, WK_W8_128, WK_X2_64, WK_X2_128, WK_R3_64, WK_R3_128 };
-struct WinoPlan { int kind, n_tail, n_main; WGeom geo; };
+struct WinoPlan { int kind, n_tail, n_main; WGeom geo; int bn_slots, bn_ptcut; };
 
 int wino_cu_count() {
     int ncu = 256, dev = 0;
@@ -1409,7 +1484,7 @@
 }
 
 WinoPlan wino_plan_of(int n, int cin, int h, int w, int cout, int ncu) {
-    WinoPlan p = {0, 0, 0, {}};
+    WinoPlan p = {0, 0, 0, {}, 0, 0};
     if (n <= 0 || cin <= 0 || h <= 0 || w <= 0 || cout <= 0 || cout % 4 != 0) return p;
     const long big = (long)n * (cin > cout ? cin : cout) * h * w;
     if (big >= (1l << 31)) return p;
@@ -1434,6 +1509,9 @@
         p.n_main = cut4 ? tiles4 - rem4 : tiles4;
         p.n_tail = cut4 ? rem4 * 8 * nw : 0;
         p.kind = x2 ? (cout > 64 ? WK_X2_128 : WK_X2_64) : nw == 8 ? (cout > 64 ? WK_W8_128 : WK_W8_64) : (cout > 64 ? WK_W4_128 : WK_W4_64);
+        const int co_tiles4 = cout > 64 ? vocr_cdiv(cout, 128) : 1, nseg4 = cout > 64 ? nw / 2 : nw;
+        p.bn_ptcut = p.n_main / co_tiles4;
+        p.bn_slots = p.bn_ptcut + (tiles4 / co_tiles4 - p.bn_ptcut) * 4 * nseg4;
         return p;
     }
     const bool f23 = wino2_mode() && big < (1l << 29);
@@ -1450,6 +1528,10 @@
 extern "C" int vocr_conv3x3_wino_plan(int n, int cin, int h, int w, int cout) {
     const WinoPlan p = wino_plan_of(n, cin, h, w, cout, wino_cu_count());
     return p.kind == 0 ? 0 : p.kind + (p.n_tail > 0 ? 16 : 0);
+}
+
+extern "C" int vocr_conv3x3_wino_bn_slots(int n, int cin, int h, int w, int cout) {
+    return wino_plan_of(n, cin, h, w, cout, wino_cu_count()).bn_slots;
 }
 
 extern "C" int vocr_conv3x3_wino_fwd(const float* x, const float* wpack, const float* bias, float* y, int n, int cin, int h,
@@ -1469,13 +1551,17 @@
     const float* wdirect = wpack + (size_t)cin * (f43 ? 18 : 12) * cout;
     const dim3 grid(p.n_tail + p.n_main);
     const int ct = vocr_cdiv(cout, 128);
+    VocrBnEpilogue* ep = vocr_internal_bn_epilogue();
+    double* bnp = (ep->part && bias && p.bn_slots > 0 && p.bn_slots == ep->slots) ? ep->part : nullptr;
+    ep->delivered = bnp ? 1 : 0;
+    if (!bnp) { ep->part = nullptr; ep->slots = 0; }
     switch (p.kind) {
-        case WK_X2_128: conv3x3_wino4x2_kernel_128<<<grid, 256, 0, s>>>(x, wpack, bias, y, zp, n, cin, h, w, cout, geo, ct, wdirect, p.n_tail, p.n_main); break;
-        case WK_W8_128: conv3x3_wino4w8_kernel_128<<<grid, 512, 0, s>>>(x, wpack, bias, y, zp, n, cin, h, w, cout, geo, ct, wdirect, p.n_tail, p.n_main); break;
-        case WK_W4_128: conv3x3_wino4_kernel_128<<<grid, 256, 0, s>>>(x, wpack, bias, y, zp, n, cin, h, w, cout, geo, ct, wdirect, p.n_tail, p.n_main); break;
-        case WK_X2_64: conv3x3_wino4x2_kernel_64<<<grid, 256, 0, s>>>(x, wpack, bias, y, zp, n, cin, h, w, cout, geo, 1, wdirect, p.n_tail, p.n_main); break;
-        case WK_W8_64: conv3x3_wino4w8_kernel_64<<<grid, 512, 0, s>>>(x, wpack, bias, y, zp, n, cin, h, w, cout, geo, 1, wdirect, p.n_tail, p.n_main); break;
-        case WK_W4_64: conv3x3_wino4_kernel_64<<<grid, 256, 0, s>>>(x, wpack, bias, y, zp, n, cin, h, w, cout, geo, 1, wdirect, p.n_tail, p.n_main); break;
+        case WK_X2_128: conv3x3_wino4x2_kernel_128<<<grid, 256, 0, s>>>(x, wpack, bias, y, zp, n, cin, h, w, cout, geo, ct, wdirect, p.n_tail, p.n_main, bnp); break;
+        case WK_W8_128: conv3x3_wino4w8_kernel_128<<<grid, 512, 0, s>>>(x, wpack, bias, y, zp, n, cin, h, w, cout, geo, ct, wdirect, p.n_tail, p.n_main, bnp); break;
+        case WK_W4_128: conv3x3_wino4_kernel_128<<<grid, 256, 0, s>>>(x, wpack, bias, y, zp, n, cin, h, w, cout, geo, ct, wdirect, p.n_tail, p.n_main, bnp); break;
+        case WK_X2_64: conv3x3_wino4x2_kernel_64<<<grid, 256, 0, s>>>(x, wpack, bias, y, zp, n, cin, h, w, cout, geo, 1, wdirect, p.n_tail, p.n_main, bnp); break;
+        case WK_W8_64: conv3x3_wino4w8_kernel_64<<<grid, 512, 0, s>>>(x, wpack, bias, y, zp, n, cin, h, w, cout, geo, 1, wdirect, p.n_tail, p.n_main, bnp); break;
+        case WK_W4_64: conv3x3_wino4_kernel_64<<<grid, 256, 0, s>>>(x, wpack, bias, y, zp, n, cin, h, w, cout, geo, 1, wdirect, p.n_tail, p.n_main, bnp); break;
         case WK_F23_128: conv3x3_wino2_kernel_128<<<grid, 256, 0, s>>>(x, wpack, bias, y, zp, n, cin, h, w, cout, geo, ct, wdirect, p.n_tail, p.n_main); break;
         case WK_F23_64: conv3x3_wino2_kernel_64<<<grid, 256, 0, s>>>(x, wpack, bias, y, zp, n, cin, h, w, cout, geo, 1, wdirect, p.n_tail, p.n_main); break;
         case WK_R3_128: conv3x3_wino_kernel<128><<<grid, 256, 0, s>>>(x, wpack, bias, y, zp, n, cin, h, w, cout, geo, ct, wdirect, p.n_tail, p.n_main); break;
diff --git a/vistaocr_amd/csrc/vocr_common.h b/vistaocr_amd/csrc/vocr_common.h
--- a/vistaocr_amd/csrc/vocr_common.h
+++ b/vistaocr_amd/csrc/vocr_common.h
@@ -42,6 +42,13 @@
 };
 int vocr_allow_dynamic_lds(const void* const* kernels, int n, int bytes, VocrPerDevice* done, const char* who);
 
+struct VocrBnEpilogue {
+    double* part;
+    int slots;
+    int delivered;
+};
+VocrBnEpilogue* vocr_internal_bn_epilogue();
+
 __device__ __forceinline__ float wave_sum(float v) {
 #pragma unroll
     for (int o = 32; o > 0; o >>= 1) v += __shfl_xor(v, o, 64);
diff --git a/vistaocr_amd/ops.py b/vistaocr_amd/ops.py
--- a/vistaocr_amd/ops.py
+++ b/vistaocr_amd/ops.py
@@ -236,6 +236,8 @@
 
 
 _BN_FUSED_FINAL = _exp("VOCR_BN_FUSED_FINAL", "1") == "1"
+_BN_EPILOGUE = _exp("VOCR_BN_EPILOGUE", "1") == "1"
+_BN_EPILOGUE_MIN_PIXELS = int(_exp("VOCR_BN_EPILOGUE_MIN_PIXELS", str(1 << 19)))
 _WINO = _exp("VOCR_CONV_WINO", "1") == "1"
 _WINO_WGRAD = _exp("VOCR_WGRAD_WINO", "1") == "1"
 
@@ -300,7 +302,16 @@
     return bool(_lib.load().vocr_conv3x3_wgrad_h16_supported(cin, cout))
 
 
-def conv3x3_forward(x, wpack, bias, cout):
+def _bn_epilogue_ws(slots, n, cout, hw, device):
+    if slots <= 0:
+        return None
+    lib = _lib.load()
+    ws = _ws(max(lib.vocr_bn_workspace_bytes(n, cout, hw), lib.vocr_bn_epilogue_workspace_bytes(cout, slots)), device)
+    call("vocr_bn_epilogue_arm", _p(ws), slots)
+    return ws
+
+
+def conv3x3_forward(x, wpack, bias, cout, bn_stats=False):
     n, cin, h, w = x.shape
     y = torch.empty(n, cout, h, w, dtype=torch.float32, device=x.device)
     lib = _lib.load()
@@ -313,8 +324,11 @@
         wpack = wpack[rows - 9 * cin:]
         rows = 9 * cin
     fn = "vocr_conv3x3_wino_fwd" if rows != 9 * cin else "vocr_conv3x3_fwd"
+    ws = None
+    if bn_stats and bias is not None and fn == "vocr_conv3x3_wino_fwd":
+        ws = _bn_epilogue_ws(lib.vocr_conv3x3_wino_bn_slots(n, cin, h, w, cout), n, cout, h * w, x.device)
     call(fn, _p(x), _p(wpack), _p(bias), _p(y), n, cin, h, w, cout, _stream())
-    return y
+    return (y, ws) if bn_stats else y
 
 
 def conv3x3_c1_forward(x, weight, bias, f16=False):
@@ -372,6 +386,9 @@
         lib = _lib.load()
         ctx.f16 = bool(f16)
         x16p = None
+        fused_final = training and _BN_FUSED_FINAL
+        want_ep = bool(fused_final and _BN_EPILOGUE and n * h * w >= _BN_EPILOGUE_MIN_PIXELS)
+        ws = None
         if cin == 1 and not ctx.needs_input_grad[0]:
             pf = pd = None
             y = conv3x3_c1_forward(x, weight, bias, ctx.f16)
@@ -391,14 +408,13 @@
                 pf, pd = prep.packs[weight.data_ptr()]
             else:
                 pf, pd = conv3x3_pack(weight)
-            y = conv3x3_forward(x, pf, bias, cout)
+            y, ws = conv3x3_forward(x, pf, bias, cout, bn_stats=True) if want_ep else (conv3x3_forward(x, pf, bias, cout), None)
         mean = torch.empty(cout, dtype=torch.float32, device=x.device)
         invstd = torch.empty(cout, dtype=torch.float32, device=x.device)
         xhat_sum = None
-        fused_final = training and _BN_FUSED_FINAL
-        ws = None
         if training:
-            ws = _ws(lib.vocr_bn_workspace_bytes(n, cout, h * w), x.device)
+            if ws is None:
+                ws = _ws(lib.vocr_bn_workspace_bytes(n, cout, h * w), x.device)
             xhat_sum = torch.empty(cout, dtype=torch.float32, device=x.device)
             if not fused_final:
                 call("vocr_bn_train_stats", _p(y), n, cout, h * w, eps, momentum, _p(mean), _p(invstd), _p(running_mean),
```

Result: no change. 2286 line-images/sec (-0.1%).
